# HaSai666/rec_pangu

Hardware: AMD Instinct MI355X
Metric: samples/sec DeepFM Criteo-shape bsz=65536/GPU (train step: fwd+bwd+dense Adam+zero_grad) (higher is better)
Workload: dtype f32

## Files before the change

### include/rec_pangu_hip.h

```cpp
#ifndef REC_PANGU_HIP_H
#define REC_PANGU_HIP_H

#include <stddef.h>
#include <stdint.h>

#ifdef __cplusplus
extern "C" {
#endif

#define RP_OK 0
#define RP_ERR_ARG (-1)
#define RP_ERR_LAUNCH (-2)
#define RP_ERR_UNSUPPORTED (-3)

#define RP_MAX_FIELDS 64

#define RP_ACT_NONE 0
#define RP_ACT_RELU 1
#define RP_ACT_MASK 2
#define RP_ACT_TANH 3
#define RP_ACT_SIGMOID 4
#define RP_ACT_LEAKY 5

#define RP_MATMUL_FP32 0
#define RP_MATMUL_BF16 1
#define RP_MATMUL_AUTO 2
#define RP_MATMUL_BF16X3 3
#define RP_MATMUL_BF16X6 6
int rp_set_matmul_precision(int mode);
int rp_get_matmul_precision(void);

typedef void *rp_stream_t;

#define RP_ABI_VERSION 108
int rp_version(void);
const char *rp_last_error(void);
uint64_t rp_launch_count(void);

int rp_embed_gather_fwd(const float *arena, const int64_t *row_base, const int64_t *row_count,
                        const int64_t *const *idx_ptrs, int F, const float *const *dense_ptrs, int ND,
                        int64_t B, int D, float *x, int64_t ldx, float *fm_out, float *sum_out,
                        int32_t *keys_out, int32_t *err_flag, rp_stream_t stream);

int rp_embed_gather_linear_fits(int D, int ND, int hidden, int64_t ldx, int64_t ldw);
int rp_embed_gather_linear_fwd(const float *arena, const int64_t *row_base, const int64_t *row_count,
                               const int64_t *const *idx_ptrs, int F, const float *const *dense_ptrs, int ND, int64_t B,
                               int D, float *x, int64_t ldx, const float *W, int64_t ldw, const float *bias, float *h1,
                               float *fm_out, float *sum_out, int32_t *keys_out, int32_t *err_flag, float *xd, rp_stream_t stream);
int rp_embed_gather_linear_fwd_bf16(const void *arena_bf16, const int64_t *row_base, const int64_t *row_count,
                                    const int64_t *const *idx_ptrs, int F, const float *const *dense_ptrs, int ND, int64_t B,
                                    int D, const float *W, int64_t ldw, const float *bias, float *h1, float *fm_out,
                                    void *x_bf16, int64_t ldx, float *sum_out, int32_t *keys_out, int32_t *err_flag,
                                    float *xd, rp_stream_t stream);

int rp_sort_workspace_bytes(int64_t n, size_t *bytes);
int rp_sort_pairs_i32(void *workspace, size_t workspace_bytes, const int32_t *keys_in, int32_t *keys_out,
                      int32_t *pos_out, int64_t n, int end_bit, rp_stream_t stream);
int rp_sort_pairs_fields_workspace_bytes(int64_t B, int F, size_t *bytes);
int rp_sort_pairs_fields_i32(void *workspace, size_t workspace_bytes, const int32_t *keys_in, int32_t *keys_out,
                             int32_t *pos_out, int64_t B, int F, const int64_t *field_base, const int64_t *field_rows,
                             rp_stream_t stream);
int rp_embed_grad_reduce_workspace_bytes(int64_t n, int D, size_t *bytes);
int rp_embed_grad_reduce(const int32_t *sorted_keys, const int32_t *sorted_pos, int64_t n, int64_t B, int D,
                         const float *dx, int64_t ldx, const float *gfm, const float *sum_in,
                         const float *arena, float *grad_arena, int accumulate, void *workspace,
                         size_t workspace_bytes, rp_stream_t stream);
int rp_embed_grad_gemm_fits(int D, int hidden, int64_t lddh, int64_t ldwt);
int rp_embed_grad_gemm(const int32_t *sorted_keys, const int32_t *sorted_pos, int64_t n, int64_t B, int D, const float *dh,
                       int64_t lddh, const float *wt, int64_t ldwt, const float *dx, int64_t ldx, const float *gfm,
                       const float *sum_in, const float *arena, float *grad_arena, int accumulate, uint64_t skip_fields,
                       void *workspace, size_t workspace_bytes, rp_stream_t stream);
int rp_embed_grad_tiny_workspace_bytes(int64_t B, size_t *bytes);
int rp_embed_grad_tiny(const int32_t *keys, int64_t B, const int32_t *tiny_field, const int64_t *tiny_base,
                       const int32_t *tiny_rows, int n_tiny, const float *dh, int64_t lddh, const float *wt, int64_t ldwt,
                       const float *gfm, const float *sum_in, const float *arena, float *grad_arena, int accumulate,
                       float *dw, int64_t lddw, void *workspace, size_t workspace_bytes, rp_stream_t stream);
int rp_embed_grad_seg_fits(int D, int hidden, int64_t lddh);
int rp_embed_grad_seg_workspace_bytes(int64_t n, int64_t B, int D, size_t *bytes);
int rp_embed_grad_seg(const int32_t *sorted_keys, const int32_t *sorted_pos, int64_t n, int64_t B, int D, const float *dh,
                      int64_t lddh, const float *w, int64_t ldw, const float *gfm, const float *sum_in, const float *arena,
                      float *grad_arena, int accumulate, uint64_t skip_fields, const int64_t *field_rows, float *dw,
                      int64_t lddw, void *workspace, size_t workspace_bytes, rp_stream_t stream);
int rp_embed_grad_ss_workspace_bytes(int64_t n, int64_t B, int D, uint64_t skip_fields, size_t *bytes);
int rp_embed_grad_ss_mark_sizes(int64_t B, int n_kept, size_t *n_rows, size_t *n_offs);
int rp_embed_grad_ss_mark(const int32_t *sorted_keys, int64_t n, int64_t B, uint64_t skip_fields, int32_t *ustart, int32_t *ukey,
                          int32_t *offs, rp_stream_t stream);
int rp_embed_grad_ss(const int32_t *sorted_keys, const int32_t *sorted_pos, int64_t n, int64_t B, int D, const float *dh,
                     int64_t lddh, const float *w, int64_t ldw, const float *gfm, const float *sum_in, const float *arena,
                     float *grad_arena, int accumulate, uint64_t skip_fields, const int64_t *field_rows, float *dw,
                     int64_t lddw, const int32_t *ustart, const int32_t *ukey, const int32_t *offs, int phases,
                     void *workspace, size_t workspace_bytes, rp_stream_t stream);
int rp_embed_grad_smp_fits(int D, int hidden, int64_t lddh);
int rp_embed_grad_smp_workspace_bytes(int64_t B, int n_fields, size_t *bytes);
int rp_embed_grad_smp_mark_scratch(int64_t B, int n_fields, size_t *n_int32);
int rp_embed_grad_smp_mark(const int32_t *sorted_keys, const int32_t *sorted_pos, int64_t n, int64_t B,
                           const int32_t *fields, int n_fields, int32_t *dupq, int32_t *dupkeys, int32_t *scratch,
                           rp_stream_t stream);
int rp_embed_grad_smp(const int32_t *keys, const int32_t *dupq, const int32_t *dupkeys, int64_t B, int F,
                      const int32_t *fields, const int64_t *field_base, const int64_t *field_rows, int n_fields,
                      const float *dh, int64_t lddh, const float *w, int64_t ldw,
                      const float *gfm, const float *sum_in, const float *arena, float *grad_arena, int accumulate,
                      float *dw, int64_t lddw, int phases, void *workspace, size_t workspace_bytes, rp_stream_t stream);
int rp_embed_grad_reduce_rows(const int32_t *keys, const float *rows, int64_t n, int D, float *grad_arena, int accumulate,
                              void *workspace, size_t workspace_bytes, rp_stream_t stream);
int rp_zero_rows(const int32_t *keys, int64_t n, int D, float *grad_arena, rp_stream_t stream);
int rp_fill_words(void *dst, int64_t n_words, uint32_t value, rp_stream_t stream);

int rp_linear_fwd(const float *a, int64_t lda, const float *w, int64_t ldw, const float *bias, float *out,
                  int64_t ldo, int64_t M, int N, int K, int act, const float *aux, int64_t ldaux,
                  rp_stream_t stream);
int rp_linear_wgrad_workspace_bytes(int64_t M, int N, int K, size_t *bytes);
int rp_linear_wgrad(const float *dy, int64_t lddy, const float *x, int64_t ldx, float *dw, int64_t lddw,
                    float *db, int64_t M, int N, int K, int accumulate, void *workspace,
                    size_t workspace_bytes, rp_stream_t stream);
int rp_linear_wgrad_xbf16(const float *dy, int64_t lddy, const void *x_bf16, int64_t ldx, float *dw, int64_t lddw,
                          float *db, int64_t M, int N, int K, int accumulate, void *workspace, size_t workspace_bytes,
                          rp_stream_t stream);
int rp_transpose(const float *in, int64_t ldin, float *out, int64_t ldout, int R, int C, int C_out, rp_stream_t stream);
int rp_transpose_copy(const float *in, int64_t ldin, float *out, int64_t ldout, int R, int C, int C_out, float *copy,
                      int64_t ldcopy, rp_stream_t stream);
int rp_copy_rows(const float *in, int64_t ldin, float *out, int64_t ldout, int R, int C, rp_stream_t stream);
int rp_add_rows(const float *in, int64_t ldin, float *out, int64_t ldout, int R, int C, rp_stream_t stream);
int64_t rp_pieces_ld(int K, int np);
int rp_pieces_pack(const float *in, int64_t ld, int64_t M, int K, int np, void *out, int64_t ldo, rp_stream_t stream);
int rp_linear_fwd_pieces(const void *a, int64_t lda, const void *w, int64_t ldw, const float *bias, float *out,
                         int64_t ldo, int64_t M, int N, int K, int np, int act, const float *aux, int64_t ldaux,
                         rp_stream_t stream);
int rp_relu_bwd(const float *dy, int64_t lddy, const float *act_out, int64_t ldact, float *out, int64_t ldo,
                int64_t M, int N, rp_stream_t stream);
int rp_act_fwd(const float *x, int64_t ldx, float *y, int64_t ldy, int64_t M, int N, int act, rp_stream_t stream);
int rp_act_bwd(const float *dy, int64_t lddy, const float *act_out, int64_t ldact, float *out, int64_t ldo, int64_t M,
               int N, int act, rp_stream_t stream);

int rp_crossnet_fwd(const float *x0, int64_t ldx, int d, int L, const float *W, const float *Bv, const float *wfc,
                    const float *bfc, float *xout, int64_t ldo, float *logit, float *s_out, int64_t B,
                    rp_stream_t stream);

int rp_cin_layer_fwd(const float *x0, int64_t ld0, const float *xp, int64_t ldp, const float *W, const float *bias,
                     float *out, float *pooled, int64_t ldpool, int H, int M, int O, int D, int64_t B,
                     rp_stream_t stream);
int rp_cin_layer_bwd_x(const float *x0, int64_t ld0, const float *xp, int64_t ldp, const float *W, const float *g_out,
                       const float *g_pool, int64_t ldgp, float *dx0, int64_t lddx0, int add_dx0, float *dxp,
                       int64_t lddxp, int H, int M, int O, int D, int64_t B, rp_stream_t stream);
int rp_cin_layer_bwd_w_workspace_bytes(int64_t B, int H, int M, int O, size_t *bytes);
int rp_cin_layer_bwd_w(const float *x0, int64_t ld0, const float *xp, int64_t ldp, const float *g_out,
                       const float *g_pool, int64_t ldgp, float *dW, float *dbias, int H, int M, int O, int D,
                       int64_t B, void *workspace, size_t workspace_bytes, rp_stream_t stream);

int rp_field_attention_fits(int T, int Din, int H, int a, int has_res);
int rp_field_attention_fwd(const float *x, int64_t ldx, const float *W, int T, int Din, int H, int a, int has_res,
                           float scale, float *out, int64_t B, rp_stream_t stream);
int rp_field_attention_bwd_workspace_bytes(int64_t B, int T, int Din, int H, int a, int has_res, size_t *bytes);
int rp_field_attention_bwd(const float *x, int64_t ldx, const float *W, int T, int Din, int H, int a, int has_res,
                           float scale, const float *gout, float *dx, int64_t lddx, float *dW, int64_t B,
                           void *workspace, size_t workspace_bytes, rp_stream_t stream);

int rp_mmoe_combine_fwd(const float *z, int64_t ldz, int K, int E, int T, float *out, float *gate, int64_t B,
                        rp_stream_t stream);
int rp_mmoe_combine_bwd(const float *z, int64_t ldz, int K, int E, int T, const float *gate, const float *dout,
                        float *dz, int64_t lddz, int64_t B, rp_stream_t stream);

int rp_crossnet_bwd_rows(const float *x0, int64_t ldx, int d, int L, const float *W, const float *wfc,
                         const float *s_in, const float *g_x, int64_t ldg, const float *g_logit, float *dx0,
                         int64_t lddx, float *V, int64_t B, rp_stream_t stream);
int rp_crossnet_param_grads(const float *P, int64_t ldp, const float *cs, const float *W, const float *Bv, const float *wfc,
                            const float *colg, int L, int d, float *dW, float *dB, float *dwfc, rp_stream_t stream);

int rp_cin_bs_fits(int H, int M, int D);
int rp_accumulate(float *dst, const float *src, int64_t n, rp_stream_t stream);
int rp_cin_bs_fwd(const float *x0, int64_t ld0, const float *xp, int64_t ldp, const void *wp, const float *bias, int H,
                  int M, int O, int D, float *out, float *pooled, int64_t B, rp_stream_t stream);
int rp_cin_bs_bwd_x(const float *xk, int64_t ldk, const void *wp, const float *gout, const float *gpool, int R, int Cn,
                    int O, int D, float *dx, int64_t lddx, int64_t B, rp_stream_t stream);
int rp_cin_bs_bwd_w_workspace_bytes(int64_t B, int O, size_t *bytes);
int rp_cin_bs_bwd_w(const float *x0, int64_t ld0, const float *xp, int64_t ldp, const float *gout, const float *gpool,
                    int H, int M, int O, int D, float *dW, float *db, int64_t B, void *workspace, size_t workspace_bytes,
                    rp_stream_t stream);
int rp_cin_pair_fits(int H, int O, int D);
int rp_cin_pair_fwd(const float *x0, int64_t ld0, const void *wsp, const float *bias, int H, int O, int D, float *out,
                    float *pooled, int64_t B, rp_stream_t stream);
int rp_cin_pair_bwd_x(const float *x0, int64_t ld0, const void *wst, const float *gout, const float *gpool,
                      const int32_t *lstart, const int32_t *lent, int H, int O, int D, float *dx, int64_t lddx, int64_t B,
                      int accumulate, rp_stream_t stream);
int rp_cin_pair_bwd_w_workspace_bytes(int64_t B, int H, int O, size_t *bytes);
int rp_cin_pair_bwd_w(const float *x0, int64_t ld0, const float *gout, const float *gpool, int H, int O, int D, float *dW,
                      float *db, int64_t B, void *workspace, size_t workspace_bytes, rp_stream_t stream);

int rp_cin_last_fits(int H, int M, int D);
int rp_cin_last_fwd(const float *x0, int64_t ld0, const float *xp, int64_t ldp, const float *vt, int H, int M, int D,
                    float *pooled, int64_t B, rp_stream_t stream);
int rp_cin_last_bwd_x(const float *x0, int64_t ld0, const float *xp, int64_t ldp, const float *vt, const float *g, int H,
                      int M, int D, float *dx0, int64_t ldd0, float *dxp, int64_t lddp, int64_t B, rp_stream_t stream);
int rp_cin_last_bwd_v_workspace_bytes(int64_t B, int H, int M, size_t *bytes);
int rp_cin_last_bwd_v(const float *x0, int64_t ld0, const float *xp, int64_t ldp, const float *g, int H, int M, int D,
                      float *dV, int64_t B, void *workspace, size_t workspace_bytes, rp_stream_t stream);
int rp_cin_pair_pieces(const float *W, int O, int H, void *wsp, void *wst, rp_stream_t stream);
int rp_cin_head_params_fwd(const float *WL, const float *bL, const float *c, int O, int H, int M, float *vt, float *vb,
                           rp_stream_t stream);
int rp_cin_head_params_bwd(const float *WL, const float *bL, const float *c, const float *dV, const float *sg, float Dscale,
                           int O, int H, int M, float *dWL, float *dbL, float *dc, rp_stream_t stream);
int rp_add_scalars(float *out, int64_t n, const float *a, float scale, const float *b0, rp_stream_t stream);
int rp_sum_all(const float *x, int64_t n, float *out, rp_stream_t stream);

// ... 336 lines not shown
```

### rec_pangu_amd/csrc/common.h

```cpp
#pragma once
#include <hip/hip_runtime.h>
#include <stdint.h>
#include <stddef.h>
#include "../../include/rec_pangu_hip.h"

#include <string.h>
#include <tuple>
#include <utility>

int rp_fail(int code, const char *fmt, ...);
void rp_count_launch();

#define RP_MAX_KERNARG 4096
bool rp_plan_recording();
void rp_plan_record(const void *func, dim3 grid, dim3 block, unsigned shmem, hipStream_t stream, const char *blob,
                    size_t blob_bytes, const size_t *offsets, int nargs);

template <typename T>
static inline size_t rp_pack_arg(char *buf, size_t &off, const T &v) {
    off = (off + alignof(T) - 1) & ~(size_t)(alignof(T) - 1);
    const size_t at = off;
    memcpy(buf + at, &v, sizeof(T));
    off += sizeof(T);
    return at;
}

template <size_t I, typename K, typename Tup>
static inline K rp_arg_or_zero(Tup &t) {
    if constexpr (I < std::tuple_size<Tup>::value) return static_cast<K>(std::get<I>(t));
    else return K{};
}

template <typename... KArgs, typename Tup, size_t... I>
static inline void rp_launch_packed(void (*kernel)(KArgs...), dim3 grid, dim3 block, unsigned shmem, hipStream_t stream,
                                    Tup &args, std::index_sequence<I...>) {
    constexpr int N = (int)sizeof...(KArgs);
    static_assert((sizeof(KArgs) + ... + 0) + 16 * sizeof...(KArgs) <= RP_MAX_KERNARG, "kernel arguments exceed the packing buffer");
    alignas(16) char buf[RP_MAX_KERNARG];
    size_t off = 0;
    size_t offs[N ? N : 1] = {rp_pack_arg<KArgs>(buf, off, rp_arg_or_zero<I, KArgs>(args))...};
    void *ptrs[N ? N : 1];
    for (int i = 0; i < N; ++i) ptrs[i] = buf + offs[i];
    if (rp_plan_recording()) rp_plan_record(reinterpret_cast<const void *>(kernel), grid, block, shmem, stream, buf, off, offs, N);
    (void)hipLaunchKernel(reinterpret_cast<const void *>(kernel), grid, block, ptrs, shmem, stream);
}

template <typename... KArgs, typename... Args>
static inline void rp_launch(void (*kernel)(KArgs...), dim3 grid, dim3 block, unsigned shmem, hipStream_t stream,
                             Args &&...args) {
    static_assert(sizeof...(Args) <= sizeof...(KArgs), "kernel launch: too many arguments");
    auto tup = std::forward_as_tuple(std::forward<Args>(args)...);
    rp_launch_packed(kernel, grid, block, shmem, stream, tup, std::make_index_sequence<sizeof...(KArgs)>());
}

#undef hipLaunchKernelGGL
#define hipLaunchKernelGGL(kernel, grid, block, shmem, stream, ...) rp_launch(kernel, grid, block, shmem, stream, __VA_ARGS__)

#define RP_REQUIRE(cond, ...)                                  \
    do {                                                       \
        if (!(cond)) return rp_fail(RP_ERR_ARG, __VA_ARGS__);  \
    } while (0)

#define RP_LAUNCH_CHECK(name)                                                        \
    do {                                                                             \
        hipError_t e__ = hipGetLastError();                                          \
        if (e__ != hipSuccess)                                                       \
            return rp_fail(RP_ERR_LAUNCH, "%s: %s", name, hipGetErrorString(e__));   \
        rp_count_launch();                                                           \
    } while (0)

static inline bool rp_aligned16(const void *p) { return (reinterpret_cast<uintptr_t>(p) & 15u) == 0; }
static inline int64_t rp_cdiv(int64_t a, int64_t b) { return (a + b - 1) / b; }

typedef float f32x4 __attribute__((ext_vector_type(4)));
typedef float f32x16 __attribute__((ext_vector_type(16)));

__device__ __forceinline__ float rp_act_apply(int act, float v) {
    switch (act) {
        case RP_ACT_RELU: return v > 0.f ? v : 0.f;
        case RP_ACT_TANH: return tanhf(v);
        case RP_ACT_SIGMOID: return 1.f / (1.f + expf(-v));
        case RP_ACT_LEAKY: return v > 0.f ? v : 0.01f * v;
        default: return v;
    }
}
__device__ __forceinline__ float rp_act_grad(int act, float dy, float y) {
    switch (act) {
        case RP_ACT_RELU: return y > 0.f ? dy : 0.f;
        case RP_ACT_TANH: return dy * (1.f - y * y);
        case RP_ACT_SIGMOID: return dy * (y * (1.f - y));
        case RP_ACT_LEAKY: return y > 0.f ? dy : 0.01f * dy;
        default: return dy;
    }
}

#define RP_WAVE 64

int rp_matmul_products(double flops, double bytes);

int rp_int_grad_reduce_finish(int64_t n, int D, int64_t nb0, char *wbase, float *piece0, int32_t *key0, float *grad_arena,
                              int accumulate, hipStream_t s);
```

### rec_pangu_amd/csrc/embed.hip

```cpp
#include "common.h"
#include <cstdlib>
#include "bfsplit.h"

struct IdxPtrs {
    const int64_t *p[RP_MAX_FIELDS];
};
struct DensePtrs {
    const float *p[RP_MAX_FIELDS];
};

template <int VEC>
struct Vec;
template <>
struct Vec<4> {
    typedef f32x4 T;
    static __device__ __forceinline__ T load(const float *p) { return *reinterpret_cast<const f32x4 *>(p); }
    static __device__ __forceinline__ void store(float *p, T v) { *reinterpret_cast<f32x4 *>(p) = v; }
    static __device__ __forceinline__ T zero() { return f32x4{0.f, 0.f, 0.f, 0.f}; }
    static __device__ __forceinline__ float hsum(T v) { return (v.x + v.y) + (v.z + v.w); }
};
template <>
struct Vec<1> {
    typedef float T;
    static __device__ __forceinline__ T load(const float *p) { return *p; }
// ... 150 lines not shown
                    gs = 0.f;
                    run_head = true;
                }
            }
        }
        __syncthreads();
        if (grp == 0) {
            const bool head_open = pkey[0][0] >= 0;
            int last_g = -1;
            for (int g2 = GPB - 1; g2 >= 0; --g2)
                if (pkey[g2][0] >= 0 || pkey[g2][1] >= 0) {
                    last_g = g2;
                    break;
                }
            const int64_t wg_end = ((int64_t)blockIdx.x + 1) * GPB * RP_SEG;
            const int last_active = (int)(((n < wg_end ? n : wg_end) - (int64_t)blockIdx.x * GPB * RP_SEG + RP_SEG - 1) / RP_SEG) - 1;
            const bool tail_open = last_g >= 0 && last_g == last_active && pcont[last_g] != 0;
            int32_t cur = -1;
            bool cur_is_head = false;
            typename V::T cacc = V::zero();
            int32_t headkey = -1, tailkey = -1;
            typename V::T headv = V::zero(), tailv = V::zero();
            for (int g2 = 0; g2 < GPB; ++g2) {
#pragma unroll
                for (int slot = 0; slot < 2; ++slot) {
                    const int32_t key = pkey[g2][slot];
                    if (key < 0) continue;
                    const typename V::T pv = V::load(&piece[g2][slot][t * VEC]);
                    if (key == cur) {
                        cacc += pv;
                    } else {
                        if (cur >= 0) {
                            if (cur_is_head) {
                                headkey = cur;
                                headv = cacc;
                            } else if (col_ok) {
                                float *dst = G + (int64_t)cur * D + c;
                                V::store(dst, accumulate ? V::load(dst) + cacc : cacc);
                            }
                        }
                        cur = key;
                        cacc = pv;
                        cur_is_head = head_open && g2 == 0 && slot == 0;
                    }
                }
            }
            if (cur >= 0) {
                if (tail_open) {
                    if (cur_is_head) {
                        headkey = cur;
                        headv = cacc;
                        tailkey = cur;
                    } else {
                        tailkey = cur;
                        tailv = cacc;
                    }
                } else if (cur_is_head) {
                    headkey = cur;
                    headv = cacc;
                } else if (col_ok) {
                    float *dst = G + (int64_t)cur * D + c;
                    V::store(dst, accumulate ? V::load(dst) + cacc : cacc);
                }
            }
            if (col_ok) {
                V::store(hp + c, headv);
                V::store(tp + c, tailv);
            }
            if (t == 0 && c0 == 0) {
                gkey[2 * (int64_t)blockIdx.x] = headkey;
                gkey[2 * (int64_t)blockIdx.x + 1] = tailkey;
            }
        }
        __syncthreads();
    }
}

#define EG_LD 72
#define EG_CT 68
#define EGL_MAXF 32

#define EGL_XLD 68
#define EGL_KLD 33
template <bool FULL, bool STORE_X = true, bool BF16_ROWS = false>
__global__ __launch_bounds__(256, 2) void embed_gather_linear_kernel(
    const float *__restrict__ arena, const int64_t *__restrict__ row_base, const int64_t *__restrict__ row_count,
    IdxPtrs idx, int F, DensePtrs dense, int ND, int64_t B, int64_t blk0, float *__restrict__ x, int64_t ldx,
    const float *__restrict__ W, int64_t ldw, const float *__restrict__ bias, float *__restrict__ h1,
    float *__restrict__ fm_out, float *__restrict__ sum_out, int32_t *__restrict__ keys_out, int32_t *__restrict__ err_flag,
    float *__restrict__ xd) {
    constexpr int D = 64;
    __shared__ __attribute__((aligned(16))) __bf16 Wt[3][64][EG_LD];
    __shared__ __attribute__((aligned(16))) float Xs[128][EGL_XLD];
    __shared__ int32_t Ks[128][EGL_KLD];
    const int t = threadIdx.x;
    const int wv = t >> 6, l = t & 63, i = l & 31, h = l >> 5;
    const int64_t blk = blk0 + blockIdx.x;
    const int64_t b = blk * 128 + 32 * wv + i;
    const bool bok = FULL || b < B;
    const int64_t bc = bok ? b : B - 1;
    const int g = t >> 4, sub = t & 15;
    const int wd = t >> 2, wc = (t & 3) * 16;

    for (int f = h; f < F; f += 2) {
        int64_t id = idx.p[f][bc];
        if (id < 0 || id >= row_count[f]) {
            if (bok) *err_flag = 1;
            id = 0;
        }
        const int64_t key = row_base[f] + id;
        Ks[32 * wv + i][f] = (int32_t)key;
        if (keys_out != nullptr && bok) keys_out[(int64_t)f * B + b] = (int32_t)key;
    }
    __syncthreads();
    const int g8 = t >> 3, s8 = t & 7;
    auto row_of = [&](int u) { return BF16_ROWS ? g8 + 32 * (u >> 1) : g + 16 * u; };
    auto col_of = [&](int u) { return BF16_ROWS ? 8 * s8 + 4 * (u & 1) : 4 * sub; };
    auto load_rows = [&](int f, f32x4 (&v)[8]) {
        if (BF16_ROWS) {
#pragma unroll
            for (int u = 0; u < 4; ++u) {
                const uint4 w4 = *reinterpret_cast<const uint4 *>(reinterpret_cast<const uint16_t *>(arena) +
                                                                  (int64_t)Ks[g8 + 32 * u][f] * D + 8 * s8);
                v[2 * u] = f32x4{__uint_as_float(w4.x << 16), __uint_as_float(w4.x & 0xffff0000u),
                                 __uint_as_float(w4.y << 16), __uint_as_float(w4.y & 0xffff0000u)};
                v[2 * u + 1] = f32x4{__uint_as_float(w4.z << 16), __uint_as_float(w4.z & 0xffff0000u),
                                     __uint_as_float(w4.w << 16), __uint_as_float(w4.w & 0xffff0000u)};
            }
        } else {
#pragma unroll
            for (int u = 0; u < 8; ++u) v[u] = *reinterpret_cast<const f32x4 *>(arena + (int64_t)Ks[g + 16 * u][f] * D + 4 * sub);
        }
    };
    auto load_w = [&](int col0, f32x4 (&v)[4]) {
        const float *src = W + (int64_t)wd * ldw + col0 + wc;
#pragma unroll
        for (int u = 0; u < 4; ++u) v[u] = *reinterpret_cast<const f32x4 *>(src + 4 * u);
    };
    f32x16 acc[2];
#pragma unroll
    for (int nt = 0; nt < 2; ++nt)
#pragma unroll
        for (int r = 0; r < 16; ++r) acc[nt][r] = 0.f;
    f32x4 S[8];
    float q[8];
#pragma unroll
    for (int u = 0; u < 8; ++u) {
        S[u] = f32x4{0.f, 0.f, 0.f, 0.f};
        q[u] = 0.f;
    }
    f32x4 cur[8], nxt[8], wq[4], wqn[4];
    load_rows(0, cur);
    load_w(0, wq);
    for (int f = 0; f < F; ++f) {
        const int fn = f + 1 < F ? f + 1 : f;
        load_rows(fn, nxt);
        load_w(fn * D, wqn);
        __syncthreads();
#pragma unroll
        for (int u = 0; u < 8; ++u) {
            const int r = row_of(u);
            *reinterpret_cast<f32x4 *>(&Xs[r][col_of(u)]) = cur[u];
            const int64_t br = blk * 128 + r;
            if (STORE_X && (FULL || (x != nullptr && br < B))) {
                if (BF16_ROWS) {
                    uint2 w2;
                    w2.x = (__float_as_uint(cur[u][0]) >> 16) | (__float_as_uint(cur[u][1]) & 0xFFFF0000u);
                    w2.y = (__float_as_uint(cur[u][2]) >> 16) | (__float_as_uint(cur[u][3]) & 0xFFFF0000u);
                    *reinterpret_cast<uint2 *>(reinterpret_cast<uint16_t *>(x) + br * ldx + (int64_t)f * D + col_of(u)) = w2;
                } else {
                    *reinterpret_cast<f32x4 *>(x + br * ldx + (int64_t)f * D + col_of(u)) = cur[u];
                }
            }
            S[u] += cur[u];
#pragma unroll
            for (int e = 0; e < 4; ++e) q[u] = __builtin_fmaf(cur[u][e], cur[u][e], q[u]);
        }
#pragma unroll
        for (int u = 0; u < 2; ++u) {
            f32x8 v;
#pragma unroll
            for (int e = 0; e < 4; ++e) {
                v[e] = wq[2 * u][e];
                v[4 + e] = wq[2 * u + 1][e];
            }
            bf16x8 pc[3];
            bf_split8<3>(v, pc);
#pragma unroll
            for (int qq = 0; qq < 3; ++qq) *reinterpret_cast<bf16x8 *>(&Wt[qq][wd][wc + 8 * u]) = pc[qq];
        }
        __syncthreads();
#pragma unroll
        for (int ks = 0; ks < 4; ++ks) {
            const f32x4 v0 = *reinterpret_cast<const f32x4 *>(&Xs[32 * wv + i][ks * 16 + 8 * h]);
            const f32x4 v1 = *reinterpret_cast<const f32x4 *>(&Xs[32 * wv + i][ks * 16 + 8 * h + 4]);
            f32x8 av;
#pragma unroll
            for (int e = 0; e < 4; ++e) {
                av[e] = v0[e];
                av[4 + e] = v1[e];
            }
            bf16x8 a[3];
            bf_split8<3>(av, a);
#pragma unroll
            for (int nt = 0; nt < 2; ++nt) {
                bf16x8 bq[3];
#pragma unroll
                for (int qq = 0; qq < 3; ++qq) bq[qq] = *reinterpret_cast<const bf16x8 *>(&Wt[qq][nt * 32 + i][ks * 16 + 8 * h]);
#pragma unroll
                for (int pr = 0; pr < 6; ++pr) {
                    if (BF16_ROWS && BfProd<6>::pa(pr) != 0) continue;
                    acc[nt] = __builtin_amdgcn_mfma_f32_32x32x16_bf16(a[BfProd<6>::pa(pr)], bq[BfProd<6>::pb(pr)], acc[nt], 0, 0, 0);
                }
            }
        }
#pragma unroll
        for (int u = 0; u < 8; ++u) cur[u] = nxt[u];
#pragma unroll
        for (int u = 0; u < 4; ++u) wq[u] = wqn[u];
    }
    if (ND > 0) {
        __syncthreads();
        {
#pragma unroll
            for (int u = 0; u < 4; ++u) {
                const int e = (t & 3) * 4 + u;
                const float v = e < ND ? W[(int64_t)wd * ldw + (int64_t)F * D + e] : 0.f;
                const __bf16 hi = (__bf16)v;
                const float r1 = v - (float)hi;
                const __bf16 mid = (__bf16)r1;
                Wt[0][wd][e] = hi;
                Wt[1][wd][e] = mid;
                Wt[2][wd][e] = (__bf16)(r1 - (float)mid);
            }
        }
        f32x8 dv;
#pragma unroll
        for (int e = 0; e < 8; ++e) {
            const int k = 8 * h + e;
            dv[e] = k < ND ? dense.p[k][bc] : 0.f;
        }
        __syncthreads();
        if (x != nullptr && bok && BF16_ROWS) {
            uint16_t *xt = reinterpret_cast<uint16_t *>(x) + b * ldx + (int64_t)F * D;
#pragma unroll
            for (int e = 0; e < 8; ++e)
                if (8 * h + e < ND) {
                    uint32_t ub = __float_as_uint(dv[e]);
                    ub += 0x7FFFu + ((ub >> 16) & 1u);
                    xt[8 * h + e] = (uint16_t)(ub >> 16);
                }
            for (int64_t j = (int64_t)F * D + ND + h; j < ldx; j += 2) reinterpret_cast<uint16_t *>(x)[b * ldx + j] = 0;
        } else if (x != nullptr && bok) {
            float *xt = x + b * ldx + (int64_t)F * D;
#pragma unroll
            for (int e = 0; e < 8; ++e)
                if (8 * h + e < ND) xt[8 * h + e] = dv[e];
            for (int64_t j = (int64_t)F * D + ND + h; j < ldx; j += 2) x[b * ldx + j] = 0.f;
        }
        if (xd != nullptr && bok) {
            float *xt = xd + b * 64;
#pragma unroll
            for (int e = 0; e < 8; ++e) xt[8 * h + e] = (8 * h + e < ND) ? dv[e] : 0.f;
            for (int j = 16 + h; j < 64; j += 2) xt[j] = 0.f;
        }
        bf16x8 a[3];
        bf_split8<3>(dv, a);
#pragma unroll
        for (int nt = 0; nt < 2; ++nt) {
            bf16x8 bq[3];
#pragma unroll
            for (int qq = 0; qq < 3; ++qq) bq[qq] = *reinterpret_cast<const bf16x8 *>(&Wt[qq][nt * 32 + i][8 * h]);
#pragma unroll
            for (int pr = 0; pr < 6; ++pr)
                acc[nt] = __builtin_amdgcn_mfma_f32_32x32x16_bf16(a[BfProd<6>::pa(pr)], bq[BfProd<6>::pb(pr)], acc[nt], 0, 0, 0);
        }
    } else {
        if (x != nullptr && bok && BF16_ROWS)
            for (int64_t j = (int64_t)F * D + h; j < ldx; j += 2) reinterpret_cast<uint16_t *>(x)[b * ldx + j] = 0;
        else if (x != nullptr && bok)
            for (int64_t j = (int64_t)F * D + h; j < ldx; j += 2) x[b * ldx + j] = 0.f;
        if (xd != nullptr && bok)
            for (int j = h; j < 64; j += 2) xd[b * 64 + j] = 0.f;
    }
#pragma unroll
    for (int nt = 0; nt < 2; ++nt) {
        const int n = nt * 32 + i;
        const float bv = bias != nullptr ? bias[n] : 0.f;
#pragma unroll
        for (int r = 0; r < 16; ++r) {
            const int64_t m = blk * 128 + 32 * wv + (r & 3) + 8 * (r >> 2) + 4 * h;
            if (FULL || m < B) h1[m * 64 + n] = fmaxf(acc[nt][r] + bv, 0.f);
        }
    }
    if (BF16_ROWS) {
#pragma unroll
        for (int u = 0; u < 4; ++u) {
            const int64_t br = blk * 128 + g8 + 32 * u;
            float fmv = -(q[2 * u] + q[2 * u + 1]);
#pragma unroll
            for (int e = 0; e < 4; ++e) {
                fmv = __builtin_fmaf(S[2 * u][e], S[2 * u][e], fmv);
                fmv = __builtin_fmaf(S[2 * u + 1][e], S[2 * u + 1][e], fmv);
            }
            fmv += __shfl_xor(fmv, 1, 64);
            fmv += __shfl_xor(fmv, 2, 64);
            fmv += __shfl_xor(fmv, 4, 64);
            if ((FULL || br < B) && fm_out != nullptr && s8 == 0) fm_out[br] = 0.5f * fmv;
            if ((FULL || br < B) && sum_out != nullptr) {
                *reinterpret_cast<f32x4 *>(sum_out + br * D + 8 * s8) = S[2 * u];
                *reinterpret_cast<f32x4 *>(sum_out + br * D + 8 * s8 + 4) = S[2 * u + 1];
            }
        }
        return;
    }
#pragma unroll
    for (int u = 0; u < 8; ++u) {
        const int64_t br = blk * 128 + g + 16 * u;
        float fmv = -q[u];
#pragma unroll
        for (int e = 0; e < 4; ++e) fmv = __builtin_fmaf(S[u][e], S[u][e], fmv);
        fmv += __shfl_xor(fmv, 1, 64);
        fmv += __shfl_xor(fmv, 2, 64);
        fmv += __shfl_xor(fmv, 4, 64);
        fmv += __shfl_xor(fmv, 8, 64);
        if (FULL || br < B) {
            if (fm_out != nullptr && sub == 0) fm_out[br] = 0.5f * fmv;
            if (sum_out != nullptr) *reinterpret_cast<f32x4 *>(sum_out + br * D + 4 * sub) = S[u];
        }
    }
}

static int embed_gather_linear_launch(const float *arena, bool bf16_rows, const int64_t *row_base, const int64_t *row_count,
                                      const int64_t *const *idx_ptrs, int F, const float *const *dense_ptrs, int ND,
                                      int64_t B, int D, float *x, int64_t ldx, const float *W, int64_t ldw,
                                      const float *bias, float *h1, float *fm_out, float *sum_out, int32_t *keys_out,
                                      int32_t *err_flag, float *xd, rp_stream_t stream);

extern "C" int rp_embed_gather_linear_fits(int D, int ND, int hidden, int64_t ldx, int64_t ldw) {
    return (D == 64 && hidden == 64 && ND >= 0 && ND <= 16 && ldx % 4 == 0 && ldw % 4 == 0) ? 1 : 0;
}

extern "C" int rp_embed_gather_linear_fwd(const float *arena, const int64_t *row_base, const int64_t *row_count,
                                          const int64_t *const *idx_ptrs, int F, const float *const *dense_ptrs, int ND,
                                          int64_t B, int D, float *x, int64_t ldx, const float *W, int64_t ldw,
                                          const float *bias, float *h1, float *fm_out, float *sum_out, int32_t *keys_out,
                                          int32_t *err_flag, float *xd, rp_stream_t stream) {
    return embed_gather_linear_launch(arena, false, row_base, row_count, idx_ptrs, F, dense_ptrs, ND, B, D, x, ldx, W, ldw, bias,
                                      h1, fm_out, sum_out, keys_out, err_flag, xd, stream);
}

extern "C" int rp_embed_gather_linear_fwd_bf16(const void *arena_bf16, const int64_t *row_base, const int64_t *row_count,
                                               const int64_t *const *idx_ptrs, int F, const float *const *dense_ptrs, int ND,
                                               int64_t B, int D, const float *W, int64_t ldw, const float *bias, float *h1,
                                               float *fm_out, void *x_bf16, int64_t ldx, float *sum_out, int32_t *keys_out,
                                               int32_t *err_flag, float *xd, rp_stream_t stream) {
    RP_REQUIRE(x_bf16 == nullptr || (ldx % 4 == 0 && (reinterpret_cast<uintptr_t>(x_bf16) & 7u) == 0),
               "embed_gather_linear_fwd_bf16: the bf16 activation needs ldx %% 4 == 0 and 8-byte alignment");
    return embed_gather_linear_launch(reinterpret_cast<const float *>(arena_bf16), true, row_base, row_count, idx_ptrs, F,
                                      dense_ptrs, ND, B, D, reinterpret_cast<float *>(x_bf16), ldx, W, ldw, bias, h1, fm_out,
                                      sum_out, keys_out, err_flag, xd, stream);
}

static int embed_gather_linear_launch(const float *arena, bool bf16_rows, const int64_t *row_base, const int64_t *row_count,
                                      const int64_t *const *idx_ptrs, int F, const float *const *dense_ptrs, int ND,
                                      int64_t B, int D, float *x, int64_t ldx, const float *W, int64_t ldw,
                                      const float *bias, float *h1, float *fm_out, float *sum_out, int32_t *keys_out,
                                      int32_t *err_flag, float *xd, rp_stream_t stream) {
    RP_REQUIRE(arena && row_base && row_count && idx_ptrs && W && h1 && err_flag, "embed_gather_linear_fwd: null pointer");
    RP_REQUIRE(!(x && xd), "embed_gather_linear_fwd: give x (full activation) or xd (dense columns only), not both");
    RP_REQUIRE(F >= 1 && F <= RP_MAX_FIELDS && B >= 0, "embed_gather_linear_fwd: bad F/B");
    RP_REQUIRE(ND == 0 || dense_ptrs, "embed_gather_linear_fwd: dense_ptrs is null with ND=%d", ND);
    RP_REQUIRE((int64_t)F * B < (int64_t)INT32_MAX, "embed_gather_linear_fwd: F*B overflows int32 positions");
    if (F > EGL_MAXF || !rp_embed_gather_linear_fits(D, ND, 64, x ? ldx : 4, ldw) || !rp_aligned16(arena) || !rp_aligned16(W) ||
        (x && (!rp_aligned16(x) || ldx < (int64_t)F * D + ND)) || ldw < (int64_t)F * D + ND ||
        (sum_out && !rp_aligned16(sum_out)))
        return rp_fail(RP_ERR_UNSUPPORTED, "embed_gather_linear_fwd: needs D = 64, a 64-wide layer, ND <= 16, aligned operands");
    if (B == 0) return RP_OK;
    IdxPtrs ip;
    DensePtrs dp;
    for (int f = 0; f < F; ++f) {
        RP_REQUIRE(idx_ptrs[f], "embed_gather_linear_fwd: idx_ptrs[%d] is null", f);
        ip.p[f] = idx_ptrs[f];
    }
    for (int j = 0; j < ND; ++j) {
        RP_REQUIRE(dense_ptrs[j], "embed_gather_linear_fwd: dense_ptrs[%d] is null", j);
        dp.p[j] = dense_ptrs[j];
    }
    const int64_t nfull = B / 128;
    const int64_t nblk = rp_cdiv(B, 128);
    hipStream_t s = (hipStream_t)stream;
    if (bf16_rows) {
        if (nfull > 0 && x != nullptr)
            hipLaunchKernelGGL((embed_gather_linear_kernel<true, true, true>), dim3((unsigned)nfull), dim3(256), 0, s, arena,
                               row_base, row_count, ip, F, dp, ND, B, (int64_t)0, x, ldx, W, ldw, bias, h1, fm_out, sum_out,
                               keys_out, err_flag, xd);
        else if (nfull > 0)
            hipLaunchKernelGGL((embed_gather_linear_kernel<true, false, true>), dim3((unsigned)nfull), dim3(256), 0, s, arena,
                               row_base, row_count, ip, F, dp, ND, B, (int64_t)0, x, ldx, W, ldw, bias, h1, fm_out, sum_out,
                               keys_out, err_flag, xd);
        if (nblk > nfull)
            hipLaunchKernelGGL((embed_gather_linear_kernel<false, true, true>), dim3((unsigned)(nblk - nfull)), dim3(256), 0, s,
                               arena, row_base, row_count, ip, F, dp, ND, B, nfull, x, ldx, W, ldw, bias, h1, fm_out, sum_out,
                               keys_out, err_flag, xd);
        RP_LAUNCH_CHECK("embed_gather_linear_fwd (bf16 rows)");
        return RP_OK;
    }
    if (nfull > 0 && x != nullptr)
        hipLaunchKernelGGL((embed_gather_linear_kernel<true, true>), dim3((unsigned)nfull), dim3(256), 0, s, arena, row_base,
                           row_count, ip, F, dp, ND, B, (int64_t)0, x, ldx, W, ldw, bias, h1, fm_out, sum_out, keys_out, err_flag,
                           xd);
    else if (nfull > 0)
        hipLaunchKernelGGL((embed_gather_linear_kernel<true, false>), dim3((unsigned)nfull), dim3(256), 0, s, arena, row_base,
                           row_count, ip, F, dp, ND, B, (int64_t)0, x, ldx, W, ldw, bias, h1, fm_out, sum_out, keys_out, err_flag,
                           xd);
    if (nblk > nfull)
        hipLaunchKernelGGL((embed_gather_linear_kernel<false, true>), dim3((unsigned)(nblk - nfull)), dim3(256), 0, s, arena,
                           row_base, row_count, ip, F, dp, ND, B, nfull, x, ldx, W, ldw, bias, h1, fm_out, sum_out, keys_out,
                           err_flag, xd);
    RP_LAUNCH_CHECK("embed_gather_linear_fwd");
    return RP_OK;
}

#define EG_MAXG 34
struct GradRanges {
    int n;
    int64_t start[EG_MAXG], end[EG_MAXG];
    int tile0[EG_MAXG];
};

template <bool FM_U>
__global__ __launch_bounds__(256, 3) void embed_grad_gemm_kernel(
    const int32_t *__restrict__ sk, const int32_t *__restrict__ sp, int64_t n, int Bi, const float *__restrict__ dh,
    int64_t lddh, const float *__restrict__ wt, int64_t ldwt, const float *__restrict__ dx, int64_t ldx,
    const float *__restrict__ gfm, const float *__restrict__ sum_in, const float *__restrict__ arena,
    float *__restrict__ G, int accumulate, float *__restrict__ gpiece, int32_t *__restrict__ gkey, GradRanges rg) {
    typedef Vec<4> V;
    constexpr int D = 64, TPR = 16, VEC = 4, GPB = 16, W = 64;
    constexpr int SM_B = 3 * 64 * EG_LD * 2, SM_C = 128 * EG_CT * 4;
    __shared__ __attribute__((aligned(16))) char smem[SM_B > SM_C ? SM_B : SM_C];
    __shared__ __attribute__((aligned(16))) float piece[GPB][2][W];
    __shared__ int32_t pkey[GPB][2];
    __shared__ int32_t pcont[GPB];
    __shared__ int32_t tkey[130];
    __shared__ int32_t tsmp[128];
    __shared__ int32_t tfld[128];
    __shared__ float tgf[128];
    typedef __bf16(*BTile)[64][EG_LD];
    BTile Bt = reinterpret_cast<BTile>(smem);
    float(*Ct)[EG_CT] = reinterpret_cast<float(*)[EG_CT]>(smem);
    const int t = threadIdx.x % TPR, grp = threadIdx.x / TPR;
    int gi = 0;
    for (int g2 = 1; g2 < rg.n; ++g2)
        if ((int)blockIdx.x >= rg.tile0[g2]) gi = g2;
    const int64_t wg0 = rg.start[gi] + (int64_t)((int)blockIdx.x - rg.tile0[gi]) * GPB * RP_SEG;
    const int64_t gend = rg.end[gi];
    {
        const int wv = threadIdx.x >> 6, l = threadIdx.x & 63, i = l & 31, h = l >> 5;
        const int64_t prow = wg0 + 32 * wv + i;
        const bool rok = prow < gend;
        const int32_t pp = rok ? sp[prow] : 0;
        const int32_t kk = rok ? sk[prow] : -1;
        if (threadIdx.x == 0) tkey[0] = wg0 > 0 ? sk[wg0 - 1] : -1;
        if (threadIdx.x == 64) tkey[129] = wg0 + 128 < n ? sk[wg0 + 128] : -1;
        const int fr = pp / Bi, br = pp - fr * Bi;
        const int64_t plast = (wg0 + 127 < gend ? wg0 + 127 : gend - 1);
        const int f_lo = __builtin_amdgcn_readfirstlane(sp[wg0] / Bi), f_hi = __builtin_amdgcn_readfirstlane(sp[plast] / Bi);
        if (h == 0) {
            tkey[1 + 32 * wv + i] = kk;
            tsmp[32 * wv + i] = br;
            tfld[32 * wv + i] = fr;
        }
        const bool wrap = __syncthreads_or(rok && (fr < f_lo || fr > f_hi)) != 0;
        const float gme = (gfm != nullptr && rok) ? gfm[br] : 0.f;
        f32x4 araw[4][2];
        const float *asrc = dh + (int64_t)br * lddh + 8 * h;
#pragma unroll
        for (int ks = 0; ks < 4; ++ks) {
            araw[ks][0] = *reinterpret_cast<const f32x4 *>(asrc + ks * 16);
            araw[ks][1] = *reinterpret_cast<const f32x4 *>(asrc + ks * 16 + 4);
        }
        float uraw[2][16];
        if (FM_U) {
#pragma unroll
            for (int r = 0; r < 16; ++r) {
                const float *src = sum_in + (int64_t)tsmp[32 * wv + (r & 3) + 8 * (r >> 2) + 4 * h] * D + i;
                uraw[0][r] = src[0];
                uraw[1][r] = src[32];
            }
        }
        if (h == 0) tgf[32 * wv + i] = gme;
        f32x16 acc[2];
#pragma unroll
        for (int nt = 0; nt < 2; ++nt)
#pragma unroll
            for (int r = 0; r < 16; ++r) acc[nt][r] = 0.f;
        const int wd = threadIdx.x >> 2, wc = (threadIdx.x & 3) * 16;
        const int f_from = wrap ? 0 : f_lo, f_to = wrap ? (int)((n - 1) / Bi) : f_hi;
        bool first_pass = true, need_init = FM_U;
        for (int f = f_from; f <= f_to; ++f) {
            if (wrap && !__syncthreads_or(rok && fr == f)) continue;
// ... 1003 lines not shown
```

### rec_pangu_amd/csrc/gemm.hip

```cpp
#include "common.h"
#include <cstdlib>

#define BM 128
#define BN 64
#define BK 32
#define LDS_LD 36

__device__ __forceinline__ f32x4 load4_guard(const float *p, int valid, bool vec) {
    if (vec && valid >= 4) return *reinterpret_cast<const f32x4 *>(p);
    f32x4 v = {0.f, 0.f, 0.f, 0.f};
    if (valid > 0) v.x = p[0];
    if (valid > 1) v.y = p[1];
    if (valid > 2) v.z = p[2];
    if (valid > 3) v.w = p[3];
    return v;
}

template <bool VEC_A, bool VEC_W>
__global__ __launch_bounds__(256) void linear_fwd_kernel(const float *__restrict__ A, int64_t lda,
                                                         const float *__restrict__ W, int64_t ldw,
                                                         const float *__restrict__ bias, float *__restrict__ C,
                                                         int64_t ldc, int64_t M, int N, int K, int act,
                                                         const float *__restrict__ aux, int64_t ldaux) {
    __shared__ __attribute__((aligned(16))) float smem[(BM + BN) * LDS_LD];
// ... 826 lines not shown
#pragma unroll
        for (int p = 0; p < PF; ++p) load_tile_full((int64_t)p * TN_BM, ry[p], rx[p]);
        const int64_t nloop = (nstf - PF) / PF;
        for (int64_t it = 0; it < nloop; ++it) {
#pragma unroll
            for (int p = 0; p < PF; ++p) {
                stage(ry[p], rx[p]);
                load_tile_full((it * PF + p + PF) * TN_BM, ry[p], rx[p]);
                compute();
            }
        }
        sbeg = nloop * PF;
    } else {
#pragma unroll
        for (int p = 0; p < PF; ++p)
            if (p < nst) load_tile(mbeg + (int64_t)p * TN_BM, ry[p], rx[p]);
    }
    for (int64_t s0 = sbeg; s0 < nst; s0 += PF) {
#pragma unroll
        for (int p = 0; p < PF; ++p) {
            const int64_t st = s0 + p;
            if (st >= nst) break;
            stage(ry[p], rx[p]);
            if (st + PF < nst) load_tile(mbeg + (st + PF) * TN_BM, ry[p], rx[p]);
            compute();
        }
    }
    float *Pz = P + (int64_t)bz * N * K;
#pragma unroll
    for (int u = 0; u < NA; ++u)
#pragma unroll
        for (int kk = 0; kk < 2; ++kk) {
            const int k = k0 + kt + kk * 32 + i;
            if (k >= K) continue;
#pragma unroll
            for (int r = 0; r < 16; ++r) {
                const int n = n0 + nt + 32 * u + (r & 3) + 8 * (r >> 2) + 4 * h;
                if (n < N) Pz[(int64_t)n * K + k] = acc[u][kk][r];
            }
        }
    if (do_bias) {
#pragma unroll
        for (int u = 0; u < NA; ++u) bred[o][c + 64 * u] = bsum[u];
        __syncthreads();
        for (int e = t; e < BNT; e += 256)
            if (n0 + e < N) Pb[(int64_t)bz * N + n0 + e] = (bred[0][e] + bred[1][e]) + (bred[2][e] + bred[3][e]);
    }
}

__global__ __launch_bounds__(256) void wgrad_reduce_kernel(const float *__restrict__ P, const float *__restrict__ Pb,
                                                           int S, int N, int K, float *__restrict__ dw,
                                                           int64_t lddw, float *__restrict__ db, int accumulate) {
    __shared__ float red[16][17];
    const int c = threadIdx.x & 15, q = threadIdx.x >> 4;
    const int64_t e = (int64_t)blockIdx.x * 16 + c;
    const int64_t nk = (int64_t)N * K;
    const bool is_w = e < nk, is_b = !is_w && e < nk + N && db != nullptr;
    float s = 0.f;
    if (is_w) {
#pragma unroll 4
        for (int z = q; z < S; z += 16) s += P[(int64_t)z * nk + e];
    } else if (is_b) {
        const int n = (int)(e - nk);
#pragma unroll 4
        for (int z = q; z < S; z += 16) s += Pb[(int64_t)z * N + n];
    }
    red[q][c] = s;
    __syncthreads();
    if (q != 0) return;
#pragma unroll
    for (int j = 1; j < 16; ++j) s += red[j][c];
    if (is_w) {
        const int n = (int)(e / K), k = (int)(e - (int64_t)n * K);
        float *d = dw + (int64_t)n * lddw + k;
        *d = accumulate ? (*d + s) : s;
    } else if (is_b) {
        const int n = (int)(e - nk);
        db[n] = accumulate ? (db[n] + s) : s;
    }
}

__global__ __launch_bounds__(256) void transpose_kernel(const float *__restrict__ in, int64_t ldin,
                                                        float *__restrict__ out, int64_t ldout, int R, int C, int C_out,
                                                        float *__restrict__ copy = nullptr, int64_t ldcopy = 0) {
    __shared__ float tile[32][33];
    const int tx = threadIdx.x & 31, ty = threadIdx.x >> 5;
    const int c0 = blockIdx.x * 32, r0 = blockIdx.y * 32;
#pragma unroll
    for (int j = 0; j < 32; j += 8) {
        const int r = r0 + ty + j, c = c0 + tx;
        const bool ok = r < R && c < C;
        const float v = ok ? in[(int64_t)r * ldin + c] : 0.f;
        tile[ty + j][tx] = v;
        if (copy != nullptr && ok) copy[(int64_t)r * ldcopy + c] = v;
    }
    __syncthreads();
#pragma unroll
    for (int j = 0; j < 32; j += 8) {
        const int c = c0 + ty + j, r = r0 + tx;
        if (r < R && c < C_out) out[(int64_t)c * ldout + r] = tile[tx][ty + j];
    }
}

__global__ __launch_bounds__(256) void relu_bwd_kernel(const float *__restrict__ dy, int64_t lddy,
                                                       const float *__restrict__ y, int64_t ldy,
                                                       float *__restrict__ out, int64_t ldo, int64_t M, int N) {
    const int64_t total = M * N;
    for (int64_t e = (int64_t)blockIdx.x * blockDim.x + threadIdx.x; e < total; e += (int64_t)gridDim.x * blockDim.x) {
        const int64_t m = e / N;
        const int n = (int)(e - m * N);
        out[m * ldo + n] = (y[m * ldy + n] > 0.f) ? dy[m * lddy + n] : 0.f;
    }
}

template <int NPROD>
static void launch_smallk_rowadd(const float *a, int64_t lda, const float *w, int64_t ldw, float *out, int64_t ldo,
                                 int64_t M, int N, int K, const float *rs, const float *radd, int64_t ldadd, int nadd,
                                 hipStream_t s) {
    const int64_t mb = M / 128;
    const int tiles = N / BN;
    int64_t ysplit = rp_cdiv(768, mb);
    if (ysplit > tiles) ysplit = tiles;
    if (ysplit < 1) ysplit = 1;
    const int per = (int)rp_cdiv(tiles, ysplit);
    dim3 grid((unsigned)mb, (unsigned)rp_cdiv(tiles, per));
    hipLaunchKernelGGL((linear_fwd_bf16_smallk_kernel<NPROD, RP_ACT_NONE, true, true>), grid, dim3(256), 0, s, a, lda, w, ldw,
                       nullptr, out, ldo, M, N, K, nullptr, 0, per, rs, radd, ldadd, nadd);
}

static int g_matmul_precision = RP_MATMUL_AUTO;

extern "C" int rp_set_matmul_precision(int mode) {
    RP_REQUIRE(mode == RP_MATMUL_FP32 || mode == RP_MATMUL_BF16 || mode == RP_MATMUL_BF16X3 || mode == RP_MATMUL_BF16X6 ||
                   mode == RP_MATMUL_AUTO, "set_matmul_precision: unknown mode %d", mode);
    g_matmul_precision = mode;
    return RP_OK;
}

int rp_matmul_products(double flops, double bytes) {
    switch (g_matmul_precision) {
        case RP_MATMUL_FP32: return 0;
        case RP_MATMUL_BF16: return 1;
        case RP_MATMUL_BF16X3: return 3;
        case RP_MATMUL_BF16X6: return 6;
        default: break;
    }
    return (bytes > 0 && flops * 3.0 / bytes > 312.0) ? 3 : 6;
}

static int linear_mode(int64_t M, int N, int K) {
    if (g_matmul_precision != RP_MATMUL_AUTO) return g_matmul_precision;
    return rp_matmul_products(2.0 * M * N * K, 4.0 * ((double)M * K + (double)N * K + (double)M * N)) == 3
               ? RP_MATMUL_BF16X3 : RP_MATMUL_BF16X6;
}

extern "C" int rp_get_matmul_precision(void) { return g_matmul_precision; }

extern "C" int rp_linear_fwd_rowadd(const float *a, int64_t lda, const float *w, int64_t ldw, float *out, int64_t ldo,
                                    int64_t M, int N, int K, const float *row_scale, const float *row_add,
                                    int64_t ld_add, int add_cols, rp_stream_t stream) {
    RP_REQUIRE(a && w && out && row_scale && row_add, "linear_fwd_rowadd: null pointer");
    RP_REQUIRE(lda >= K && ldw >= K && ldo >= N && ld_add >= 64, "linear_fwd_rowadd: leading dimension too small");
    const int mode = linear_mode(M, N, K);
    const bool ok = mode != RP_MATMUL_FP32 && K >= 4 && K <= 64 && K % 4 == 0 && M >= 128 && M % 128 == 0 && N >= 64 &&
                    N % 64 == 0 && add_cols >= 0 && add_cols % 64 == 0 && add_cols <= N && lda % 4 == 0 && ldw % 4 == 0 &&
                    rp_aligned16(a) && rp_aligned16(w);
    if (!ok) return rp_fail(RP_ERR_UNSUPPORTED, "linear_fwd_rowadd: shape/alignment/mode outside the fused kernel");
    hipStream_t s = (hipStream_t)stream;
// ... 175 lines not shown
        RP_LAUNCH_CHECK("linear_wgrad partial (bf16 split)");
    } else {
#define CALL(VY, VX)                                                                                                \
    hipLaunchKernelGGL((linear_wgrad_partial_kernel<VY, VX>), grid, dim3(256), 0, s, dy, lddy, x, ldx, P, Pb, M, N, K, \
                       rows)
    if (vy && vx) CALL(true, true);
    else if (vy) CALL(true, false);
    else if (vx) CALL(false, true);
    else CALL(false, false);
#undef CALL
    RP_LAUNCH_CHECK("linear_wgrad partial");
    }
    const int64_t total = (int64_t)N * K + N;
    hipLaunchKernelGGL(wgrad_reduce_kernel, dim3((unsigned)rp_cdiv(total, 16)), dim3(256), 0, s, P, Pb, S, N, K, dw,
                       lddw, db, accumulate);
    RP_LAUNCH_CHECK("linear_wgrad reduce");
    return RP_OK;
}

extern "C" int rp_linear_wgrad_xbf16(const float *dy, int64_t lddy, const void *x_bf16, int64_t ldx, float *dw, int64_t lddw,
                                     float *db, int64_t M, int N, int K, int accumulate, void *workspace,
                                     size_t workspace_bytes, rp_stream_t stream) {
    RP_REQUIRE(dy && x_bf16 && dw && workspace, "linear_wgrad_xbf16: null pointer");
    RP_REQUIRE(M >= 1 && N >= 1 && K >= 1, "linear_wgrad_xbf16: bad M/N/K");
    RP_REQUIRE(lddy >= N && ldx >= K && lddw >= K, "linear_wgrad_xbf16: leading dimension too small");
    const int mode = linear_mode(M, N, K);
    if (mode == RP_MATMUL_FP32 || wgrad_wide(N) || ldx % 2 != 0 || (reinterpret_cast<uintptr_t>(x_bf16) & 3u) != 0)
        return rp_fail(RP_ERR_UNSUPPORTED, "linear_wgrad_xbf16: bf16 matrix-core modes, N <= 128, ldx even, 4-byte aligned x only");
    size_t need = 0;
    rp_linear_wgrad_workspace_bytes(M, N, K, &need);
    RP_REQUIRE(workspace_bytes >= need, "linear_wgrad_xbf16: workspace %zu < %zu bytes", workspace_bytes, need);
    int S;
    int64_t rows;
    wgrad_plan(M, N, K, &S, &rows);
    float *P = reinterpret_cast<float *>((reinterpret_cast<uintptr_t>(workspace) + 255) & ~(uintptr_t)255);
    float *Pb = P + (size_t)S * N * K;
    dim3 gridb((unsigned)rp_cdiv(K, TN_BK), (unsigned)rp_cdiv(N, TN_BN), (unsigned)S);
    hipStream_t s = (hipStream_t)stream;
    const float *xf = reinterpret_cast<const float *>(x_bf16);
#define CALLX(NPROD)                                                                                                       \
    hipLaunchKernelGGL((linear_wgrad_bf16_kernel<NPROD, 1, 1, true, true>), gridb, dim3(256), 0, s, dy, lddy, xf, ldx, P, Pb, M, \
                       N, K, rows, 0, 0, S)
    if (mode == RP_MATMUL_BF16X6) CALLX(6);
    else if (mode == RP_MATMUL_BF16X3) CALLX(3);
    else CALLX(1);
#undef CALLX
    RP_LAUNCH_CHECK("linear_wgrad_xbf16 partial");
    const int64_t total = (int64_t)N * K + N;
    hipLaunchKernelGGL(wgrad_reduce_kernel, dim3((unsigned)rp_cdiv(total, 16)), dim3(256), 0, s, P, Pb, S, N, K, dw, lddw, db,
                       accumulate);
    RP_LAUNCH_CHECK("linear_wgrad_xbf16 reduce");
    return RP_OK;
}

extern "C" int rp_transpose(const float *in, int64_t ldin, float *out, int64_t ldout, int R, int C, int C_out,
                            rp_stream_t stream) {
    RP_REQUIRE(in && out && R >= 1 && C >= 1 && C_out >= C && ldin >= C && ldout >= R, "transpose: bad argument");
    dim3 grid((unsigned)rp_cdiv(C_out, 32), (unsigned)rp_cdiv(R, 32));
    hipLaunchKernelGGL(transpose_kernel, grid, dim3(256), 0, (hipStream_t)stream, in, ldin, out, ldout, R, C, C_out);
    RP_LAUNCH_CHECK("transpose");
    return RP_OK;
}

__global__ __launch_bounds__(256) void copy_rows_kernel(const float *__restrict__ in, int64_t ldin, float *__restrict__ out,
                                                        int64_t ldout, int R, int C) {
    const int64_t total = (int64_t)R * C;
    for (int64_t e = (int64_t)blockIdx.x * 256 + threadIdx.x; e < total; e += (int64_t)gridDim.x * 256) {
        const int64_t r = e / C;
        const int c = (int)(e - r * C);
        out[r * ldout + c] = in[r * ldin + c];
    }
}

extern "C" int rp_transpose_copy(const float *in, int64_t ldin, float *out, int64_t ldout, int R, int C, int C_out,
                                 float *copy, int64_t ldcopy, rp_stream_t stream) {
    RP_REQUIRE(in && out && copy && R >= 1 && C >= 1 && C_out >= C && ldin >= C && ldout >= R && ldcopy >= C,
               "transpose_copy: bad argument");
    const dim3 grid((unsigned)rp_cdiv(C_out, 32), (unsigned)rp_cdiv(R, 32));
    hipLaunchKernelGGL(transpose_kernel, grid, dim3(256), 0, (hipStream_t)stream, in, ldin, out, ldout, R, C, C_out, copy, ldcopy);
    RP_LAUNCH_CHECK("transpose_copy");
    return RP_OK;
}

extern "C" int rp_copy_rows(const float *in, int64_t ldin, float *out, int64_t ldout, int R, int C, rp_stream_t stream) {
    RP_REQUIRE(in && out && R >= 1 && C >= 1 && ldin >= C && ldout >= C, "copy_rows: bad argument");
    int64_t blocks = rp_cdiv((int64_t)R * C, 256);
    if (blocks > 2048) blocks = 2048;
    hipLaunchKernelGGL(copy_rows_kernel, dim3((unsigned)blocks), dim3(256), 0, (hipStream_t)stream, in, ldin, out, ldout, R, C);
    RP_LAUNCH_CHECK("copy_rows");
    return RP_OK;
}

__global__ __launch_bounds__(256) void add_rows_kernel(const float *__restrict__ in, int64_t ldin, float *__restrict__ out,
                                                       int64_t ldout, int R, int C) {
    const int64_t total = (int64_t)R * C;
    for (int64_t e = (int64_t)blockIdx.x * 256 + threadIdx.x; e < total; e += (int64_t)gridDim.x * 256) {
        const int64_t r = e / C;
        const int c = (int)(e - r * C);
        out[r * ldout + c] += in[r * ldin + c];
    }
}

extern "C" int rp_add_rows(const float *in, int64_t ldin, float *out, int64_t ldout, int R, int C, rp_stream_t stream) {
    RP_REQUIRE(in && out && R >= 1 && C >= 1 && ldin >= C && ldout >= C, "add_rows: bad argument");
    int64_t blocks = rp_cdiv((int64_t)R * C, 256);
    if (blocks > 4096) blocks = 4096;
    hipLaunchKernelGGL(add_rows_kernel, dim3((unsigned)blocks), dim3(256), 0, (hipStream_t)stream, in, ldin, out, ldout, R, C);
    RP_LAUNCH_CHECK("add_rows");
    return RP_OK;
}

__global__ __launch_bounds__(256) void act_fwd_kernel(const float *__restrict__ x, int64_t ldx, float *__restrict__ y,
                                                      int64_t ldy, int64_t M, int N, int act) {
    const int64_t total = M * N;
    for (int64_t e = (int64_t)blockIdx.x * 256 + threadIdx.x; e < total; e += (int64_t)gridDim.x * 256) {
        const int64_t r = e / N;
        const int c = (int)(e - r * N);
        y[r * ldy + c] = rp_act_apply(act, x[r * ldx + c]);
    }
}

__global__ __launch_bounds__(256) void act_bwd_kernel(const float *__restrict__ dy, int64_t lddy, const float *__restrict__ ya,
                                                      int64_t ldact, float *__restrict__ out, int64_t ldo, int64_t M, int N,
                                                      int act) {
    const int64_t total = M * N;
    for (int64_t e = (int64_t)blockIdx.x * 256 + threadIdx.x; e < total; e += (int64_t)gridDim.x * 256) {
        const int64_t r = e / N;
        const int c = (int)(e - r * N);
        out[r * ldo + c] = rp_act_grad(act, dy[r * lddy + c], ya[r * ldact + c]);
    }
}

static bool act_kind_ok(int act) { return act == RP_ACT_RELU || act == RP_ACT_TANH || act == RP_ACT_SIGMOID || act == RP_ACT_LEAKY; }

extern "C" int rp_act_fwd(const float *x, int64_t ldx, float *y, int64_t ldy, int64_t M, int N, int act, rp_stream_t stream) {
    RP_REQUIRE(x && y && M >= 0 && N >= 1 && ldx >= N && ldy >= N && act_kind_ok(act), "act_fwd: bad argument");
    if (M == 0) return RP_OK;
    int64_t blocks = rp_cdiv(M * N, 256);
    if (blocks > 4096) blocks = 4096;
    hipLaunchKernelGGL(act_fwd_kernel, dim3((unsigned)blocks), dim3(256), 0, (hipStream_t)stream, x, ldx, y, ldy, M, N, act);
    RP_LAUNCH_CHECK("act_fwd");
    return RP_OK;
}

extern "C" int rp_act_bwd(const float *dy, int64_t lddy, const float *act_out, int64_t ldact, float *out, int64_t ldo,
                          int64_t M, int N, int act, rp_stream_t stream) {
    RP_REQUIRE(dy && act_out && out && M >= 0 && N >= 1 && act_kind_ok(act), "act_bwd: bad argument");
    if (M == 0) return RP_OK;
    int64_t blocks = rp_cdiv(M * N, 256);
    if (blocks > 4096) blocks = 4096;
    hipLaunchKernelGGL(act_bwd_kernel, dim3((unsigned)blocks), dim3(256), 0, (hipStream_t)stream, dy, lddy, act_out, ldact, out, ldo,
                       M, N, act);
    RP_LAUNCH_CHECK("act_bwd");
    return RP_OK;
}

extern "C" int rp_relu_bwd(const float *dy, int64_t lddy, const float *act_out, int64_t ldact, float *out,
                           int64_t ldo, int64_t M, int N, rp_stream_t stream) {
    RP_REQUIRE(dy && act_out && out && M >= 0 && N >= 1, "relu_bwd: bad argument");
    if (M == 0) return RP_OK;
    int64_t blocks = rp_cdiv(M * N, 256);
    if (blocks > 4096) blocks = 4096;
    hipLaunchKernelGGL(relu_bwd_kernel, dim3((unsigned)blocks), dim3(256), 0, (hipStream_t)stream, dy, lddy, act_out,
                       ldact, out, ldo, M, N);
    RP_LAUNCH_CHECK("relu_bwd");
    return RP_OK;
// ... 2 lines not shown
```

### rec_pangu_amd/functional.py

```python
import contextlib
import os
from typing import List, NamedTuple, Optional, Sequence, Tuple

import torch

from . import hip

ACT_NONE, ACT_RELU, ACT_MASK = hip.ACT_NONE, hip.ACT_RELU, hip.ACT_MASK
ACT_TANH, ACT_SIGMOID, ACT_LEAKY = hip.ACT_TANH, hip.ACT_SIGMOID, hip.ACT_LEAKY


def act_code(module):
    import torch.nn as nn
    if isinstance(module, nn.ReLU):
        return ACT_RELU
    if isinstance(module, nn.Tanh):
        return ACT_TANH
    if isinstance(module, nn.Sigmoid):
        return ACT_SIGMOID
    if isinstance(module, nn.LeakyReLU) and abs(module.negative_slope - 0.01) < 1e-12:
        return ACT_LEAKY
    return None


def _unit_inner(t: torch.Tensor) -> torch.Tensor:
    if t.dim() == 2 and (t.shape[1] <= 1 or t.stride(1) == 1) and (t.shape[0] <= 1 or t.stride(0) >= t.shape[1]):
        return t
    return t.contiguous()


def padded(width: int, pad_to: int) -> int:
    return width if pad_to <= 1 else (width + pad_to - 1) // pad_to * pad_to


def _wide_rows_grad(rows: torch.Tensor, used: int) -> Optional[torch.Tensor]:
    return hip.zeros(tuple(rows.shape), torch.float32, rows.device) if rows.shape[1] > used else None


def _rows16(w: torch.Tensor) -> torch.Tensor:
    K = w.shape[1]
    if K % 4 == 0 or K <= 64 or not w.is_cuda:
        return w
    key = (w.data_ptr(), w._version, hip.weight_epoch(), torch.cuda.is_current_stream_capturing())
    hit = getattr(w, "_rp_rows16", None)
    if hit is not None and hit[0] == key:
        return hit[1]
    with torch.no_grad():
        if w.dtype is torch.float32:
            out = hip.copy_rows(w.detach(), (K + 3) // 4 * 4)
        else:
            buf = torch.empty((w.shape[0], (K + 3) // 4 * 4), dtype=w.dtype, device=w.device)
            buf[:, :K].copy_(w)
            out = buf[:, :K]
    if not key[3]:
        try:
            w._rp_rows16 = (key, out)
        except AttributeError:
            pass
    return out


class FMFold:
    __slots__ = ("ssum", "ncols", "dfm", "folded", "dgrad", "D", "fused", "extra")

    def __init__(self, ssum, ncols, D=0):
        self.ssum, self.ncols, self.dfm, self.folded = ssum, ncols, None, False
        self.extra = None
        self.dgrad, self.D, self.fused = None, D, False


class _TokenView(torch.autograd.Function):

    @staticmethod
    def forward(ctx, x, F: int, D: int, link):
        x = _unit_inner(x)
        out = torch.empty((x.shape[0], F * D), dtype=torch.float32, device=x.device)
        hip.copy_rows_to(x[:, :F * D], out)
        ctx.link = link
        return out.view(x.shape[0], F, D)

    @staticmethod
    def backward(ctx, dtok):
        ctx.link.extra = dtok.reshape(dtok.shape[0], -1).contiguous()
        return None, None, None, None


def token_view(x, F: int, D: int, link):
    return _TokenView.apply(x, F, D, link)


class _StackRows(torch.autograd.Function):

    @staticmethod
    def forward(ctx, *ws):
        rows = [w.shape[0] for w in ws]
        out = torch.empty((sum(rows), ws[0].shape[1]), dtype=torch.float32, device=ws[0].device)
        dst, r0 = [], 0
        for r in rows:
            dst.append(out[r0:r0 + r])
            r0 += r
        src = [w.detach().contiguous() for w in ws]
        if not hip.multi_copy(dst, src):
            torch._foreach_copy_(dst, src)
        ctx.rows = rows
        return out

    @staticmethod
    def backward(ctx, g):
        g = g.contiguous()
        outs, r0 = [], 0
        for r in ctx.rows:
            outs.append(g[r0:r0 + r])
            r0 += r
        return tuple(outs)


def stack_rows(ws):
    return _StackRows.apply(*ws)


class _GradTap(torch.autograd.Function):

    @staticmethod
    def forward(ctx, t, link):
        ctx.link = link
        return t.view_as(t)

    @staticmethod
    def backward(ctx, g):
        ctx.link.dfm = g
        return g, None


def tap_fm_grad(fm, link):
    return _GradTap.apply(fm, link)


class ReluLink:
    __slots__ = ("dx",)
# ... 1245 lines not shown
        store._presorted = None
        row_base, row_count = meta if meta is not None else (store.row_base, store.row_count)
        x, fm, ssum, keys = hip.embed_gather_fwd(store.arena, row_base, row_count, idx, dense, ldx,
                                                 want_fm, want_fm and need_grad, need_grad and pre is None,
                                                 store.err_flag)
        ctx.store, ctx.want_fm, ctx.B = store, want_fm, idx[0].shape[0]
        ctx.link = store._fm_link = FMFold(ssum, len(idx) * store.embedding_dim, store.embedding_dim) \
            if (need_grad and meta is None) else None
        ctx.presorted = pre if need_grad else None
        if pre is not None:
            keys = pre.keys if need_grad else None
        ctx.save_for_backward(keys, ssum)
        if want_fm:
            return x, fm
        return x

    @staticmethod
    def backward(ctx, dx, dfm=None):
        keys, ssum = ctx.saved_tensors
        store = ctx.store
        fused = None
        if ctx.link is not None and ctx.link.dgrad is not None:
            fused, ctx.link.dgrad = ctx.link.dgrad, None
            ctx.link.fused = True
            if dx is not None and dx.dim() == 2 and dx.stride(0) == 0 and dx.stride(1) == 0:
                dx = None
        if dx is not None:
            dx = _unit_inner(dx)
        if ctx.link is not None and ctx.link.extra is not None:
            extra, ctx.link.extra = ctx.link.extra, None
            if fused is not None and dx is None and extra.shape[1] == len(store.emb_feature) * store.embedding_dim:
                dx = extra
            elif dx is None or fused is not None:
                raise RuntimeError("token_view: the gathered activation needs a consumer that materialises its gradient")
            else:
                hip.add_rows_to(extra, dx[:, :extra.shape[1]])
        gfm = dfm.contiguous() if (ctx.want_fm and dfm is not None) else None
        if ctx.link is not None and ctx.link.folded:
            ssum = None
        if fused is None:
            store.accumulate_grad(keys, ctx.B, dx, gfm, ssum, presorted=ctx.presorted)
        else:
            g = store.first_layer_grad(keys, ctx.B, *fused, gfm, ssum, presorted=ctx.presorted, dx=dx)
            if g.forms.tiny:
                g.tiny()
            g.gemm()
            g.done()
        return (None,) * (6 + len(store.emb_feature))


_WGRAD_STREAMS: dict = {}


def _side2_stream(device):
    st = _WGRAD_STREAMS.get(device)
    if st is None:
        st = _WGRAD_STREAMS[device] = hip.make_side_stream(device)
    return st


def _masked_by_consumer(lk, dy) -> bool:
    masked = lk is not None and lk.dx is not None and lk.dx.data_ptr() == dy.data_ptr() and lk.dx.shape == dy.shape
    if lk is not None:
        lk.dx = None
    return masked


def _wgrad_stream(device):
    if os.environ.get("RP_WGRAD_OVERLAP", "1") == "0" or torch.cuda.is_current_stream_capturing():
        return None
    return _side2_stream(device)


class _EmbedGatherLinear(torch.autograd.Function):

    @staticmethod
    def forward(ctx, store, idx, dense, ldx: int, weight, bias, out_link, shadow, *tables):
        pre = store._presorted
        store._presorted = None
        need_grad = any(ctx.needs_input_grad[8:])
        need_w = ctx.needs_input_grad[4] or (bias is not None and ctx.needs_input_grad[5])
        B, K, Kg = idx[0].shape[0], weight.shape[1], len(idx) * store.embedding_dim
        wt = None
        if need_grad and weight.is_cuda and weight.dtype is torch.float32 and K % 4 != 0 and K > 64:
            with torch.no_grad():
                wt, w16 = hip.transpose_copy(weight.detach(), rows_out=ldx, ld_copy=(K + 3) // 4 * 4)
        else:
            w16 = _rows16(weight)
        ctx.wt = wt
        if shadow is not None:
            want_keys = pre is None
            seg16 = (need_grad and need_w and K > Kg and len(idx) <= 64 and os.environ.get("RP_GRAD_SEG", "1") != "0"
                     and weight.shape[0] == 64 and store.embedding_dim == 64)
            x, h1, fm, ssum, keys = hip.embed_gather_linear_fwd_bf16(shadow, store.row_base, store.row_count, idx, dense, w16, bias,
                                                                     store.err_flag, train_ldx=ldx, want_keys=want_keys,
                                                                     dense_only=seg16)
            ctx.store, ctx.B, ctx.K, ctx.out_link, ctx.has_bias = store, B, K, out_link, bias is not None
            ctx.ldx, ctx.x_mode, ctx.Kg, ctx.need_tables = ldx, ("seg" if seg16 else "bf16"), Kg, need_grad
            ctx.presorted = pre if need_grad else None
            if pre is not None:
                keys = pre.keys
            ctx.save_for_backward(keys, ssum, x, h1, weight)
            store._fm_link = None
            return h1, fm
        if not need_w:
            x_mode = "none"
        elif (need_grad and K > Kg and len(idx) <= 64 and os.environ.get("RP_GRAD_SEG", "1") != "0"
              and store.embedding_dim == 64 and weight.shape[0] == 64):
            x_mode = "seg"
        else:
            x_mode = "full"
        want_keys = need_grad and pre is None
        x, h1, fm, ssum, keys = hip.embed_gather_linear_fwd(store.arena, store.row_base, store.row_count, idx, dense, ldx, w16,
                                                            bias, True, need_grad, want_keys, store.err_flag,
                                                            x_mode="dense" if x_mode == "seg" else x_mode)
        ctx.store, ctx.B, ctx.K, ctx.out_link, ctx.has_bias = store, B, K, out_link, bias is not None
        ctx.ldx, ctx.x_mode, ctx.Kg, ctx.need_tables = ldx, x_mode, Kg, need_grad
        ctx.presorted = pre if need_grad else None
        if pre is not None:
            keys = pre.keys if need_grad else None
        ctx.save_for_backward(keys, ssum, x, h1, weight)
        store._fm_link = None
        return h1, fm

    @staticmethod
    def backward(ctx, dh1, dfm):
        keys, ssum, x, h1, weight = ctx.saved_tensors
        store = ctx.store
        dh1 = _unit_inner(dh1)
        dpre = dh1 if _masked_by_consumer(ctx.out_link, dh1) else hip.relu_bwd(dh1, h1)
        dw = db = None
        need_w = ctx.needs_input_grad[4] or (ctx.has_bias and ctx.needs_input_grad[5])
        need_t = keys is not None and ctx.need_tables
        if need_w and ctx.x_mode == "none":
            raise RuntimeError("the fused lookup + first layer stored no activation (the forward ran without gradients for the "
                               "layer's weight)")
        seg = need_w and ctx.x_mode == "seg"
        dw_seg = torch.empty((64, ctx.K), dtype=torch.float32, device=dpre.device) if seg else None

        def wgrad():
            if ctx.x_mode == "seg":
                return dw_seg, hip.linear_wgrad(dpre, x, ctx.K - ctx.Kg, dw=dw_seg[:, ctx.Kg:], want_bias=ctx.has_bias)[1]
            if ctx.x_mode == "bf16":
                return hip.linear_wgrad_xbf16(dpre, x, ctx.K, want_bias=ctx.has_bias)
            return hip.linear_wgrad(dpre, x, ctx.K, want_bias=ctx.has_bias)

        wstream = _wgrad_stream(dpre.device) if (need_w and need_t) else None
        plan = hip.LaunchPlan
        in_plan = (wstream is None and need_w and need_t
                   and os.environ.get("RP_WGRAD_OVERLAP", "1") != "0" and plan.is_recording())

        def side_wgrad():
            with plan.side2(in_plan):
                out = wgrad()
                if in_plan:
                    plan.run_deferred()
            return out

        with hip.holding() if in_plan else contextlib.nullcontext():
            if wstream is not None:
                main = torch.cuda.current_stream(dpre.device)
                wstream.wait_stream(main)
                with torch.cuda.stream(wstream):
                    dw, db = wgrad()
            elif need_w and not (in_plan and seg):
                dw, db = side_wgrad()
            if need_t:
                wt = ctx.wt if ctx.wt is not None else hip.transpose(weight, rows_out=ctx.ldx)
                gfm = dfm.contiguous() if dfm is not None else None
                g = store.first_layer_grad(keys, ctx.B, dpre, wt, gfm, ssum if gfm is not None else None, presorted=ctx.presorted,
                                           w=weight if seg else None, dw=dw_seg)
                f = g.forms
                if not seg:
                    if f.tiny:
                        with plan.side2(in_plan):
                            g.tiny()
                    g.gemm()
                elif not in_plan:
                    if f.tiny:
                        g.tiny()
                    ws = g.big(1) if f.big else None
                    if f.rest:
                        g.rest()
                    if f.big:
                        g.big(2, ws)
                else:
                    if f.tiny or not f.big:
                        plan.fork2_mark()
                    if f.big:
                        ws = g.big(1)
                        if f.tiny:
                            with plan.side2():
                                g.tiny()
                            plan.side2_sync()
                        else:
                            plan.fork2_mark()
                    if f.rest:
                        g.rest()
# ... 554 lines not shown
```

### rec_pangu_amd/hip.py

```python
import contextlib
import ctypes as C
import os
import re
from typing import List, Optional, Sequence

import torch

_HERE = os.path.dirname(os.path.abspath(__file__))
HEADER_PATH = os.path.join(_HERE, os.pardir, "include", "rec_pangu_hip.h")
LIB_PATH = os.environ.get("RP_LIB_PATH") or os.path.join(_HERE, "lib", "librecpangu_hip.so")

_lib = None

_i64, _i32, _f32, _vp, _sz = C.c_int64, C.c_int, C.c_float, C.c_void_p, C.c_size_t
_f64 = C.c_double
_C_TYPES = {"int": C.c_int, "int32_t": C.c_int, "int64_t": C.c_int64, "uint32_t": C.c_uint32, "uint64_t": C.c_uint64,
            "size_t": C.c_size_t, "float": C.c_float, "double": C.c_double, "rp_stream_t": C.c_void_p}
_PROTOTYPE = re.compile(r"([A-Za-z_][\w\s]*?[\s*]+)(rp_[a-z0-9_]+)\s*\(([^()]*)\)\s*;")


def parse_header(text: str):
    text = re.sub(r"/\*.*?\*/", " ", text, flags=re.S)
    text = re.sub(r"//[^\n]*", " ", text)
    consts = {m.group(1): int(m.group(2), 0) for m in re.finditer(
# ... 208 lines not shown
    def __init__(self, name, tag=None, nbytes=0, flops=0):
        self.name = name
        self.key = name if tag is None else f"{name}[{tag}]"
        self.meta = (nbytes, flops)

    def __enter__(self):
        self.ev = None
        if _timing is not None and not _timing_paused and (_timing_only is None or self.name in _timing_only):
            self.ev = (torch.cuda.Event(enable_timing=True), torch.cuda.Event(enable_timing=True))
            self.ev[0].record()
        return self

    def __exit__(self, *exc):
        if self.ev is not None:
            self.ev[1].record()
            _timing.setdefault(self.key, []).append(self.ev)
            if self.meta != (0, 0):
                _timing_meta[self.key] = self.meta
        return False


_timing_meta = {}


def timing_summary():
    out = {}
    for name, evs in (_timing or {}).items():
        ms = [a.elapsed_time(b) for a, b in evs]
        out[name] = (len(ms), sum(ms) / max(len(ms), 1))
    return out


def timing_meta():
    return dict(_timing_meta)


_PTR_ARRAYS: dict = {}


def _ptr_array(tensors: Sequence[torch.Tensor]):
    ptrs = tuple([t.data_ptr() for t in tensors])
    arr = _PTR_ARRAYS.get(ptrs)
    if arr is None:
        for i, t in enumerate(tensors):
            if not t.is_cuda:
                raise RuntimeError(f"Expected all tensors to be on the same device: input {i} is on {t.device} but the "
                                   "model is on the HIP device (move the batch with .to(device))")
        arr = (C.c_void_p * max(len(ptrs), 1))(*ptrs)
        if len(_PTR_ARRAYS) >= 512:
            _PTR_ARRAYS.clear()
        _PTR_ARRAYS[ptrs] = arr
    return arr


def embed_gather_fwd(arena, row_base, row_count, idx: List[torch.Tensor], dense: List[torch.Tensor], ldx: int,
                     want_fm: bool, want_sum: bool, want_keys: bool, err_flag: torch.Tensor):
    _req(arena, torch.float32, "arena")
    F, ND = len(idx), len(dense)
    B, D = idx[0].shape[0], arena.shape[1]
    for t in idx:
        _req(t, torch.int64, "index")
        if t.dim() != 1 or t.shape[0] != B or not t.is_contiguous():
            raise RuntimeError("index tensors must be contiguous int64 [B]")
    for t in dense:
        _req(t, torch.float32, "dense")
        if t.dim() != 1 or t.shape[0] != B or not t.is_contiguous():
            raise RuntimeError("dense tensors must be contiguous float32 [B]")
    dev = arena.device
    x = _new((B, ldx), torch.float32, dev)
    fm = _new((B, 1), torch.float32, dev) if want_fm else None
    ssum = _new((B, D), torch.float32, dev) if want_sum else None
    keys = _new((F * B,), torch.int32, dev) if want_keys else None
    with _Timed("embed_gather_fwd", f"D={D}"):
        _check(lib().rp_embed_gather_fwd(arena.data_ptr(), row_base.data_ptr(), row_count.data_ptr(), _ptr_array(idx), F,
                                     _ptr_array(dense), ND, B, D, x.data_ptr(), ldx, _ptr(fm), _ptr(ssum), _ptr(keys),
                                     err_flag.data_ptr(), _stream()), "rp_embed_gather_fwd")
    return x, fm, ssum, keys


def embed_gather_linear_fits(D: int, F: int, ND: int, hidden: int, ldx: int, W) -> bool:
    return F <= 32 and bool(lib().rp_embed_gather_linear_fits(D, ND, hidden, ldx, _rowmajor(W, "W"))) and W.data_ptr() % 16 == 0


def embed_gather_linear_fwd(arena, row_base, row_count, idx: List[torch.Tensor], dense: List[torch.Tensor], ldx: int, W, bias,
                            want_fm: bool, want_sum: bool, want_keys: bool, err_flag: torch.Tensor, x_mode: str = "full"):
    _req(arena, torch.float32, "arena")
    _req(W, torch.float32, "W")
    F, ND = len(idx), len(dense)
    B, D = idx[0].shape[0], arena.shape[1]
    for t in idx:
        _req(t, torch.int64, "index")
        if t.dim() != 1 or t.shape[0] != B or not t.is_contiguous():
            raise RuntimeError("index tensors must be contiguous int64 [B]")
    for t in dense:
        _req(t, torch.float32, "dense")
        if t.dim() != 1 or t.shape[0] != B or not t.is_contiguous():
            raise RuntimeError("dense tensors must be contiguous float32 [B]")
    dev = arena.device
    assert x_mode in ("full", "dense", "none")
    x = _new((B, ldx), torch.float32, dev) if x_mode == "full" else None
    xd = _new((B, 64), torch.float32, dev) if x_mode == "dense" else None
    h1 = _new((B, 64), torch.float32, dev)
    fm = _new((B, 1), torch.float32, dev) if want_fm else None
    ssum = _new((B, D), torch.float32, dev) if want_sum else None
    keys = _new((F * B,), torch.int32, dev) if want_keys else None
    K = F * D + ND
    with _Timed("embed_gather_linear_fwd", f"D={D}", B * (F * (D * 4 + 8) + (F * D + ND) * 4 + 64 * 4), 2 * B * K * 64):
        _check(lib().rp_embed_gather_linear_fwd(arena.data_ptr(), row_base.data_ptr(), row_count.data_ptr(), _ptr_array(idx), F,
                                                _ptr_array(dense), ND, B, D, _ptr(x), ldx, W.data_ptr(), _rowmajor(W, "W"),
                                                _ptr(bias), h1.data_ptr(), _ptr(fm), _ptr(ssum), _ptr(keys),
                                                err_flag.data_ptr(), _ptr(xd), _stream()), "rp_embed_gather_linear_fwd")
    return (x if x_mode == "full" else xd), h1, fm, ssum, keys


def embed_gather_linear_fwd_bf16(arena_bf16, row_base, row_count, idx: List[torch.Tensor], dense: List[torch.Tensor], W, bias,
                                 err_flag: torch.Tensor, train_ldx: int = 0, want_keys: bool = False, dense_only: bool = False):
    _req(arena_bf16, torch.bfloat16, "arena_bf16")
    _req(W, torch.float32, "W")
    F, ND = len(idx), len(dense)
    B, D = idx[0].shape[0], arena_bf16.shape[1]
    dev = arena_bf16.device
    h1 = _new((B, 64), torch.float32, dev)
    fm = _new((B, 1), torch.float32, dev)
    K = F * D + ND
    if train_ldx:
        x16 = None if dense_only else _new((B, train_ldx), torch.bfloat16, dev)
        xd = _new((B, 64), torch.float32, dev) if dense_only else None
        ssum = _new((B, D), torch.float32, dev)
        keys = _new((F * B,), torch.int32, dev) if want_keys else None
        with _Timed("embed_gather_linear_fwd_bf16", f"D={D}", B * (F * (D * 2 + 8) + (F * D + ND) * 2 + 64 * 4 + D * 4), 2 * B * K * 64):
            _check(lib().rp_embed_gather_linear_fwd_bf16(arena_bf16.data_ptr(), row_base.data_ptr(), row_count.data_ptr(),
                                                         _ptr_array(idx), F, _ptr_array(dense), ND, B, D, W.data_ptr(),
                                                         _rowmajor(W, "W"), _ptr(bias), h1.data_ptr(), fm.data_ptr(),
                                                         _ptr(x16), train_ldx, ssum.data_ptr(), _ptr(keys),
                                                         err_flag.data_ptr(), _ptr(xd), _stream()), "rp_embed_gather_linear_fwd_bf16")
        return (xd if dense_only else x16), h1, fm, ssum, keys
    with _Timed("embed_gather_linear_fwd_bf16", f"D={D}", B * (F * (D * 2 + 8) + F * D * 2 + 64 * 4), 2 * B * K * 64):
        _check(lib().rp_embed_gather_linear_fwd_bf16(arena_bf16.data_ptr(), row_base.data_ptr(), row_count.data_ptr(),
                                                     _ptr_array(idx), F, _ptr_array(dense), ND, B, D, W.data_ptr(),
                                                     _rowmajor(W, "W"), _ptr(bias), h1.data_ptr(), fm.data_ptr(),
                                                     None, 0, None, None, err_flag.data_ptr(), None, _stream()),
               "rp_embed_gather_linear_fwd_bf16")
    return h1, fm


def sort_workspace(n: int, device) -> torch.Tensor:
    return _workspace("sort", n, device=device)[0]


def sort_pairs(keys: torch.Tensor, end_bit: int = 32, out=None, workspace=None):
    _req(keys, torch.int32, "keys")
    n = keys.numel()
    ws, nbytes = _workspace("sort", n, device=keys.device, given=workspace)
    assert workspace is None or ws is workspace
    ko, po = (_new_like(keys) if t is None else t for t in (out or (None, None)))
    assert ko.shape == keys.shape and po.shape == keys.shape and ko.dtype == po.dtype == torch.int32
    with _Timed("sort_pairs_i32"):
        _check(lib().rp_sort_pairs_i32(ws.data_ptr(), nbytes, keys.data_ptr(), ko.data_ptr(), po.data_ptr(), n,
                                   end_bit, _stream()), "rp_sort_pairs_i32")
    return ko, po


METRIC_AUC, METRIC_LOGLOSS = _RP["RP_METRIC_AUC"], _RP["RP_METRIC_LOGLOSS"]
METRICS_STAGES = {s: _RP["RP_METRICS_STAGE_" + s.upper()]
                  for s in ("key", "sort", "tile_sums", "tile_scan", "group_neg", "rank", "finish")}


def metrics_workspace(n: int, device) -> torch.Tensor:
    return _workspace("metrics", n, device=device)[0]


def metrics_stage_bytes(n: int, flags: int = METRIC_AUC | METRIC_LOGLOSS) -> dict:
    T = -(-n // 4096)
    auc = bool(flags & METRIC_AUC)
    out = {"key": n * (8 + (4 if auc else 0)) + 20 * T, "finish": (20 + (8 if auc else 0)) * T + 40}
    if auc:
        out.update({"sort": n * 4 * (4 * 2 + 3 + 4 * 2), "tile_sums": n * (4 + 4 + 4 + 1) + 8 * T, "tile_scan": 16 * T,
                    "group_neg": n * (4 + 1 + 4) + 8 * T, "rank": n * (4 + 1 + 4) + 12 * T})
    return out


def binary_metrics(pred: torch.Tensor, label: torch.Tensor, flags: int = METRIC_AUC | METRIC_LOGLOSS, eps: float = 1e-7,
                   workspace=None, result=None, stages=None) -> torch.Tensor:
    _req(pred, torch.float32, "pred")
    _req(label, torch.float32, "label")
    n = pred.numel()
    if label.numel() != n or not pred.is_contiguous() or not label.is_contiguous():
        raise RuntimeError("binary_metrics: pred and label must be contiguous and of one length")
    ws, _ = _workspace("metrics", n, device=pred.device, given=workspace)
    res = _new((5,), torch.int64, pred.device) if result is None else result
    sizes = metrics_stage_bytes(n, flags)
    for tag, bits in ([(None, 0)] if stages is None else [(s, METRICS_STAGES[s]) for s in stages]):
        with _Timed("binary_metrics", tag, sizes.get(tag, 0) if tag else sum(sizes.values())):
            _check(lib().rp_binary_metrics(ws.data_ptr(), ws.numel(), pred.data_ptr(), label.data_ptr(), n, eps, flags | bits,
                                           res.data_ptr(), _stream()), "rp_binary_metrics")
    return res


_SORT_FIELDS: dict = {}


def sort_fields_workspace(B: int, F: int, device) -> torch.Tensor:
    return _workspace("sort_pairs_fields", B, F, device=device)[0]


def sort_pairs_fields(keys: torch.Tensor, B: int, field_rows, out=None, workspace=None):
    _req(keys, torch.int32, "keys")
    F = len(field_rows)
    assert keys.numel() == F * B
    ck = tuple(int(r) for r in field_rows)
    arrs = _SORT_FIELDS.get(ck)
    if arrs is None:
        if len(_SORT_FIELDS) > 64:
            _SORT_FIELDS.clear()
        base, acc = [], 0
        for r in ck:
            base.append(acc)
            acc += r
        arrs = _SORT_FIELDS[ck] = ((C.c_int64 * F)(*base), (C.c_int64 * F)(*ck))
    ws, _ = _workspace("sort_pairs_fields", B, F, device=keys.device, given=workspace)
    ko, po = (_new_like(keys) if t is None else t for t in (out or (None, None)))
    assert ko.shape == keys.shape and po.shape == keys.shape and ko.dtype == po.dtype == torch.int32
    with _Timed("sort_pairs_i32"):
# ... 205 lines not shown
    _req(w, torch.float32, "w")
    lda, ldw = _rowmajor(a, "a"), _rowmajor(w, "w")
    M, N = a.shape[0], w.shape[0]
    K = w.shape[1] if K is None else K
    if a.shape[1] < K:
        raise RuntimeError(f"linear_fwd: a has {a.shape[1]} columns, need {K}")
    if out is None:
        out = _new((M, N), torch.float32, a.device)
    ldo = _rowmajor(out, "out")
    ldaux = _rowmajor(aux, "aux") if aux is not None else 0
    with _Timed("linear_fwd", f"{M}x{N}x{K}", 4 * (M * K + N * K + M * N * (2 if aux is not None else 1)), 2 * M * N * K):
        _check(lib().rp_linear_fwd(a.data_ptr(), lda, w.data_ptr(), ldw, _ptr(bias), out.data_ptr(), ldo, M, N, K, act,
                               _ptr(aux), ldaux, _stream()), "rp_linear_fwd")
    return out


def linear_fwd_rowadd(a, w, row_scale, row_add, add_cols: int, out) -> bool:
    M, K = a.shape
    N = w.shape[0]
    if not (get_matmul_precision() != "fp32" and K <= 64 and K % 4 == 0 and M % 128 == 0 and M >= 128 and N % 64 == 0
            and add_cols % 64 == 0 and 0 < add_cols <= N and row_add.shape[1] == 64 and a.stride(0) % 4 == 0
            and w.stride(0) % 4 == 0 and a.data_ptr() % 16 == 0 and w.data_ptr() % 16 == 0 and out.shape[1] >= N):
        return False
    with _Timed("linear_fwd", f"{M}x{N}x{K}+rowadd", 4 * (M * K + N * K + M * N + M * 65), 2 * M * N * K):
        _check(lib().rp_linear_fwd_rowadd(a.data_ptr(), _rowmajor(a, "a"), w.data_ptr(), _rowmajor(w, "w"), out.data_ptr(),
                                          _rowmajor(out, "out"), M, N, K, row_scale.data_ptr(), row_add.data_ptr(),
                                          _rowmajor(row_add, "row_add"), add_cols, _stream()), "rp_linear_fwd_rowadd")
    return True


def linear_wgrad(dy, x, K: int, dw=None, db=None, accumulate: bool = False, want_bias: bool = True):
    _req(dy, torch.float32, "dy")
    _req(x, torch.float32, "x")
    M, N = dy.shape
    lddy, ldx = _rowmajor(dy, "dy"), _rowmajor(x, "x")
    if dw is None:
        dw = _new((N, K), torch.float32, dy.device)
    if db is None and want_bias:
        db = _new((N,), torch.float32, dy.device)
    ws, nbytes = _workspace("linear_wgrad", M, N, K, device=dy.device)
    with _Timed("linear_wgrad", f"{M}x{N}x{K}", 4 * (M * N + M * K + N * K), 2 * M * N * K):
        _check(lib().rp_linear_wgrad(dy.data_ptr(), lddy, x.data_ptr(), ldx, dw.data_ptr(), _rowmajor(dw, "dw"), _ptr(db),
                                 M, N, K, int(accumulate), ws.data_ptr(), nbytes, _stream()), "rp_linear_wgrad")
    return dw, db


def linear_wgrad_xbf16(dy, x16, K: int, want_bias: bool = True):
    _req(dy, torch.float32, "dy")
    _req(x16, torch.bfloat16, "x16")
    M, N = dy.shape
    dw = _new((N, K), torch.float32, dy.device)
    db = _new((N,), torch.float32, dy.device) if want_bias else None
    ws, nbytes = _workspace("linear_wgrad", M, N, K, device=dy.device)
    with _Timed("linear_wgrad_xbf16", f"{M}x{N}x{K}", 4 * (M * N + N * K) + 2 * M * K, 2 * M * N * K):
        _check(lib().rp_linear_wgrad_xbf16(dy.data_ptr(), _rowmajor(dy, "dy"), x16.data_ptr(), _rowmajor(x16, "x16"),
                                           dw.data_ptr(), K, _ptr(db), M, N, K, 0, ws.data_ptr(), nbytes, _stream()),
               "rp_linear_wgrad_xbf16")
    return dw, db


def transpose(w, rows_out: Optional[int] = None):
    _req(w, torch.float32, "w")
    R, Cc = w.shape
    R4 = (R + 3) // 4 * 4
    rows = max(Cc, rows_out or 0)
    out = _new((rows, R4), torch.float32, w.device)[:, :R]
    with _Timed("transpose", f"{R}x{Cc}", 4 * (R * Cc + rows * R)):
        _check(lib().rp_transpose(w.data_ptr(), _rowmajor(w, "w"), out.data_ptr(), R4, R, Cc, rows, _stream()),
               "rp_transpose")
    return out


def transpose_copy(w, rows_out: int, ld_copy: int):
    _req(w, torch.float32, "w")
    R, Cc = w.shape
    R4 = (R + 3) // 4 * 4
    rows = max(Cc, rows_out or 0)
    out = _new((rows, R4), torch.float32, w.device)[:, :R]
    buf = _new((R, ld_copy), torch.float32, w.device)
    with _Timed("transpose_copy", f"{R}x{Cc}", 4 * (2 * R * Cc + rows * R)):
        _check(lib().rp_transpose_copy(w.data_ptr(), _rowmajor(w, "w"), out.data_ptr(), R4, R, Cc, rows, buf.data_ptr(), ld_copy,
                                       _stream()), "rp_transpose_copy")
    return out, buf[:, :Cc]


def pieces_ld(K: int, np_: int) -> int:
    return int(lib().rp_pieces_ld(int(K), int(np_)))


def pieces_pack(x, np_: int = 2, K: Optional[int] = None, out=None):
    _req(x, torch.float32, "x")
    M = x.shape[0]
    K = x.shape[1] if K is None else K
    ldo = pieces_ld(K, np_)
    if out is None:
        out = _new((M, ldo), torch.bfloat16, x.device)
    with _Timed("pieces_pack", f"{M}x{K}x{np_}", 4 * M * K + 2 * M * ldo):
        _check(lib().rp_pieces_pack(x.data_ptr(), _rowmajor(x, "x"), M, K, np_, out.data_ptr(), _rowmajor(out, "out"), _stream()),
               "rp_pieces_pack")
    return out


def linear_fwd_pieces(a_pc, w_pc, bias, K: int, np_: int = 2, act: int = ACT_NONE, aux=None, out=None):
    _req(a_pc, torch.bfloat16, "a_pc")
    _req(w_pc, torch.bfloat16, "w_pc")
    M, N = a_pc.shape[0], w_pc.shape[0]
    if out is None:
        out = _new((M, N), torch.float32, a_pc.device)
    ldaux = _rowmajor(aux, "aux") if aux is not None else 0
    with _Timed("linear_fwd_pieces", f"{M}x{N}x{K}x{np_}", 2 * (M + N) * pieces_ld(K, np_) + 4 * M * N * (2 if aux is not None else 1),
                2 * M * N * K):
        _check(lib().rp_linear_fwd_pieces(a_pc.data_ptr(), _rowmajor(a_pc, "a_pc"), w_pc.data_ptr(), _rowmajor(w_pc, "w_pc"),
                                          _ptr(bias), out.data_ptr(), _rowmajor(out, "out"), M, N, K, np_, act, _ptr(aux), ldaux,
                                          _stream()), "rp_linear_fwd_pieces")
    return out


def copy_rows(w, ld_out: int):
    _req(w, torch.float32, "w")
    R, Cc = w.shape
    buf = _new((R, ld_out), torch.float32, w.device)
    with _Timed("copy_rows", f"{R}x{Cc}", 8 * R * Cc):
        _check(lib().rp_copy_rows(w.data_ptr(), _rowmajor(w, "w"), buf.data_ptr(), ld_out, R, Cc, _stream()), "rp_copy_rows")
    return buf[:, :Cc]


def copy_rows_to(src, dst):
    _req(src, torch.float32, "src")
    _req(dst, torch.float32, "dst")
    if src.dim() != 2 or src.shape != dst.shape or src.stride(1) != 1 or dst.stride(1) != 1:
        raise RuntimeError("copy_rows_to: two 2-D tensors of one shape with unit inner stride")
    R, Cc = src.shape
    with _Timed("copy_rows", f"{R}x{Cc}", 8 * R * Cc):
        _check(lib().rp_copy_rows(src.data_ptr(), src.stride(0), dst.data_ptr(), dst.stride(0), R, Cc, _stream()), "rp_copy_rows")
    return dst


def add_rows_to(src, dst):
    _req(src, torch.float32, "src")
    _req(dst, torch.float32, "dst")
    if src.dim() != 2 or src.shape != dst.shape or src.stride(1) != 1 or dst.stride(1) != 1:
        raise RuntimeError("add_rows_to: two 2-D tensors of one shape with unit inner stride")
    R, Cc = src.shape
    with _Timed("add_rows", f"{R}x{Cc}", 12 * R * Cc):
        _check(lib().rp_add_rows(src.data_ptr(), src.stride(0), dst.data_ptr(), dst.stride(0), R, Cc, _stream()), "rp_add_rows")
    return dst


class Marker:

    def __init__(self):
        h = _vp()
        _check(lib().rp_marker_create(C.byref(h)), "rp_marker_create")
        self._h = h

    def record(self):
        _check(lib().rp_marker_record(self._h, _stream()), "rp_marker_record")

    def synchronize(self):
        _check(lib().rp_marker_wait(self._h), "rp_marker_wait")

    def __del__(self):
        try:
            if self._h is not None:
                lib().rp_marker_destroy(self._h)
        except Exception:
# ... 2149 lines not shown
```

### rec_pangu_amd/models/layers/embedding.py

```python
import copy
import os
import weakref
from types import SimpleNamespace
from typing import Dict, List, NamedTuple, Optional, Union

import torch
from torch import nn

from ... import functional as Fh
from ...grad_arena import GradArena


class SortedLookup:
    __slots__ = ("keys", "sk", "sp", "src", "versions", "sig", "event", "pinned", "workspace", "want_marks",
                 "smp_sig", "smp", "ss")

    def __init__(self, keys, sk, sp, src=None, sig=None, event=None, pinned=False, workspace=None, want_marks=True):
        self.keys, self.sk, self.sp, self.src, self.sig, self.event = keys, sk, sp, src, sig, event
        self.versions = None if src is None else tuple(t._version for t in src)
        self.pinned, self.workspace, self.want_marks = pinned, workspace, want_marks
        self.smp_sig = self.smp = self.ss = None

    def matches(self, src, sig) -> bool:
        return (self.sig == sig and len(self.src) == len(src) and all(a is b for a, b in zip(self.src, src))
# ... 381 lines not shown
            t = X[c]
            if t.dtype is not torch.int64 or t.dim() != 1 or not t.is_contiguous():
                t = t.long().reshape(-1).contiguous()
            out.append(t)
        return out

    def gather_concat(self, X, dense: List[torch.Tensor], want_fm: bool, pad_to: int = 64):
        self._ensure_packed()
        return self._gather(self._idx_list(X), None, dense, want_fm, pad_to, src=tuple(X[c] for c in self.emb_feature))

    def gather_linear_fits(self, n_dense: int, linear: nn.Linear, pad_to: int = 64) -> bool:
        from ... import hip
        F, D = len(self.emb_feature), self.embedding_dim
        d = F * D + n_dense
        ldx = Fh.padded(d, pad_to)
        w = linear.weight
        key = (id(w), w.data_ptr() % 16, tuple(w.shape), F, D, n_dense, pad_to, self._arena.is_cuda, hip.get_matmul_precision())
        hit = self.__dict__.get("_glf_cache")
        if hit is not None and hit[0] == key:
            return hit[1]
        ok = (self._arena.is_cuda and D == 64 and linear.out_features == 64 and linear.in_features == d
              and hip.get_matmul_precision() != "fp32"
              and hip.embed_gather_linear_fits(D, F, n_dense, 64, ldx, Fh._rows16(w)))
        self.__dict__["_glf_cache"] = (key, ok)
        return ok

    def bf16_lookup(self, enable: bool = True) -> None:
        if not enable:
            self._arena_bf16 = None
            return
        self._ensure_packed()
        self.flush_lazy()
        self._arena_bf16 = self._arena.detach().to(torch.bfloat16)
        self._bf16_stamp = self._bf16_stamp_now()

    def bf16_training(self, enable: bool = True) -> None:
        if not enable:
            self._shadow = None
            return
        self._ensure_packed()
        if not self._arena.is_cuda or self.embedding_dim != 64:
            raise RuntimeError("bf16_training: a HIP-resident layer with embedding_dim 64 (the fused lookup + first layer)")
        self._shadow_rebuild()

    def _shadow_rebuild(self):
        self.flush_lazy()
        self._shadow = self._arena.detach().to(torch.bfloat16)
        self._shadow_stamp = self._shadow_stamp_now()

    def _shadow_stamp_now(self):
        return (self._arena.data_ptr(), self._arena._version, tuple(p._version for p in self._tables()))

    def _shadow_for_training(self):
        sh = self.__dict__.get("_shadow")
        if sh is None:
            return None
        if sh.device != self._arena.device or sh.shape != self._arena.shape or self._shadow_stamp != self._shadow_stamp_now():
            self._shadow_rebuild()
            sh = self._shadow
        return sh

    def _bf16_stamp_now(self):
        from ... import hip
        return (self._arena._version, None if self._lazy is None else self._lazy.t, hip.weight_epoch(),
                tuple(p._version for p in self._tables()))

    def _bf16_arena_for_inference(self):
        a = self.__dict__.get("_arena_bf16")
        if a is None or torch.is_grad_enabled():
            return None
        stamp = self._bf16_stamp_now()
        if stamp != self._bf16_stamp or a.device != self._arena.device:
            raise RuntimeError("the bf16 snapshot of the embedding tables is stale (the model was trained or moved since "
                               "bf16_lookup()): call bf16_lookup() again, or bf16_lookup(False) to read the fp32 tables")
        return a

    def gather_linear(self, X, dense: List[torch.Tensor], linear: nn.Linear, out_link, pad_to: int = 64):
        self._ensure_packed()
        idx = self._idx_list(X)
        a16 = self._bf16_arena_for_inference()
        if a16 is not None:
            from ... import hip
            dense = [t.float().reshape(-1).contiguous() for t in dense]
            out = hip.embed_gather_linear_fwd_bf16(a16, self.row_base, self.row_count, idx, dense, Fh._rows16(linear.weight),
                                                   linear.bias, self.err_flag)
            if self.check_indices == "sync":
                self.raise_if_bad_index()
            return out
        F, D = len(idx), self.embedding_dim
        d = F * D + len(dense)
        ldx = Fh.padded(d, pad_to)
        dense = [t if (t.dtype is torch.float32 and t.dim() == 1 and t.is_contiguous()) else t.float().reshape(-1).contiguous()
                 for t in dense]
        src = tuple(X[c] for c in self.emb_feature)
        self._presorted = None
        shadow = self._shadow_for_training()
        if self._lazy is not None and self._lazy.t > 0:
            self._presorted = self._sorted_keys(idx, self.row_base, self.row_count, src)
            self._lazy.replay(self, self._presorted.sk)
        elif torch.is_grad_enabled():
            self._presorted = self._sorted_keys(idx, self.row_base, self.row_count, src, lookup_only=True)
        out = Fh.embed_gather_linear(self, idx, dense, ldx, linear.weight, linear.bias, out_link, shadow=shadow)
        self._start_sort_ahead()
        if self.check_indices == "sync":
            self.raise_if_bad_index()
        return out

    def _sorted_keys(self, idx, row_base, row_count, src, lookup_only: bool = False):
        from ... import hip
        sig = self._sort_sig()
        look = _find_sort(src, sig) if src is not None else None
        if look is not None:
            if look.event is not None:
                look.wait_on(torch.cuda.current_stream(self._arena.device))
            return look
        if lookup_only:
            return None
        keys = hip.embed_keys(row_base, row_count, idx, self.err_flag)
        sk, sp = self._sort_pairs(keys) if row_base is self.row_base else hip.sort_pairs(keys, end_bit=self._meta()[3])
        look = SortedLookup(keys, sk, sp, src, sig)
        if row_base is self.row_base and torch.is_grad_enabled():
            self._mark_sorted(look)
        if src is not None:
            self._cache_sort(look)
        return look

    def _sort_sig(self):
        return (self._rows_sig(), str(self._arena.device))

    @staticmethod
    def _cache_sort(look: SortedLookup) -> None:
        _SORT_CACHE.append(look)
        del _SORT_CACHE[:-4]

    def prefetch_sort(self, X) -> None:
        if self._arena.is_cuda and all(X[c].device == self._arena.device for c in self.emb_feature):
            self._ahead = X

    def _start_sort_ahead(self) -> None:
        from ... import hip
        X, self._ahead = self.__dict__.get("_ahead"), None
        if X is None:
            return
        src = tuple(X[c] for c in self.emb_feature)
        look = _find_sort(src, self._sort_sig())
        if look is not None:
            if look.pinned:
                self._sort_into(X, look)
            return
        dev = self._arena.device
        side = _side_stream(dev)
        main = torch.cuda.current_stream(dev)
        side.wait_stream(main)
        with torch.cuda.stream(side):
            idx = self._idx_list(X)
            keys = hip.embed_keys(self.row_base, self.row_count, idx, self._ahead_flag())
            look = SortedLookup(keys, *self._sort_pairs(keys), src, self._sort_sig())
            self._mark_sorted(look)
            look.event = torch.cuda.Event()
            look.event.record(side)
        for t in src:
            t.record_stream(side)
        self._cache_sort(look)

    def _ahead_flag(self):
        if self.check_indices != "sync":
            return self.err_flag
        f = self.__dict__.get("_scratch_flag")
# ... 139 lines not shown
```

### rec_pangu_amd/sharded.py

```python
import os
import weakref
from typing import Dict, List, Optional

import torch
import torch.distributed as dist
from torch import nn

from . import functional as Fh
from .grad_arena import GradArena


_STAGED: dict = {}


def _host_staged(t, group) -> bool:
    if not t.is_cuda:
        return False
    k = id(group)
    if k not in _STAGED:
        _STAGED[k] = dist.get_backend(group) == "gloo"
    return _STAGED[k]


def _recorded(fn, t) -> bool:
# ... 186 lines not shown
        self.served = (i32(world * cap), i32(world * cap))
        self.send = self.recv = [cap] * world
        self.n_unique = self.n_recv = cap * world
        self.n_requests, self.capacity, self.b = n, cap, b


class _ShardedRows(torch.autograd.Function):

    @staticmethod
    def forward(ctx, layer, keys, local_arena):
        dev = local_arena.device
        prepared, layer._prepared = layer._prepared, None
        route, recv_rows, served_sorted = prepared if prepared is not None else (None, None, None)
        if route is None:
            route = _Route(keys, layer)
        if recv_rows is None:
            recv_rows = _a2a(route.local_rows, route.recv, route.send, layer.group, layer.world)
        served = layer._local_gather(recv_rows, served_sorted, mark=bool(ctx.needs_input_grad[2]))
        ctx.presorted = getattr(layer, "_served_sorted", None)
        layer._served_sorted = None
        rows = _a2a_rows(served, route.send, route.recv, layer)
        ctx.layer, ctx.route = layer, route
        ctx.scaled, layer._scaled = layer._scaled, None
        ctx.save_for_backward(recv_rows)
        ctx.mark_non_differentiable(route.slot_of_pair, route.slot_sorted, route.pos_sorted)
        ctx.set_materialize_grads(False)
        layer._route_fm = (route.slot_fm, route.pos_fm)
        return rows, route.slot_of_pair, route.slot_sorted, route.pos_sorted

    @staticmethod
    def backward(ctx, g_rows, *_unused):
        (recv_rows,) = ctx.saved_tensors
        layer, route = ctx.layer, ctx.route
        if g_rows is None:
            return None, None, None
        prescaled = layer.world == 1 or (ctx.scaled is not None and ctx.scaled[0]) or _SEED_SCALED[0]
        g_rows = g_rows.contiguous() if prescaled else (g_rows * (1.0 / layer.world)).contiguous()
        recv_g = _a2a_rows(g_rows, route.recv, route.send, layer)
        layer._local_scatter_add(recv_rows, recv_g, presorted=ctx.presorted)
        return None, None, None


class _RowsToX(torch.autograd.Function):

    @staticmethod
    def forward(ctx, rows, slot_of_pair, dense: List[torch.Tensor], slot_sorted, pos_sorted, b: int, F: int, ldx: int,
                want_fm: bool, err_flag):
        from . import hip
        n, D = rows.shape
        dev = rows.device
        zero, cnt = _const_i64(dev, F, 0), _const_i64(dev, F, n)
        idx = [slot_of_pair[f * b:(f + 1) * b] for f in range(F)]
        x, fm, ssum, _ = hip.embed_gather_fwd(rows, zero, cnt, idx, dense, ldx, want_fm, want_fm, False, err_flag)
        ctx.cfg = (b, F, D, want_fm)
        ctx.save_for_backward(rows, slot_sorted, pos_sorted, ssum)
        return (x, fm) if want_fm else x

    @staticmethod
    def backward(ctx, dx, dfm=None):
        from . import hip
        rows, slot_sorted, pos_sorted, ssum = ctx.saved_tensors
        b, F, D, want_fm = ctx.cfg
        g_rows = hip.zeros(rows.shape, rows.dtype, rows.device)
        gfm = dfm.contiguous() if (want_fm and dfm is not None) else None
        dx = None if dx is None else Fh._unit_inner(dx)
        hip.embed_grad_reduce(slot_sorted, pos_sorted, b, D, dx, gfm, ssum if gfm is not None else None,
                              rows if gfm is not None else None, g_rows, accumulate=False)
        return g_rows, None, None, None, None, None, None, None, None, None


class _RowsToLinear(torch.autograd.Function):

    @staticmethod
    def forward(ctx, rows, slot_of_pair, dense: List[torch.Tensor], slot_sorted, pos_sorted, b: int, F: int, ldx: int,
                weight, bias, out_link, err_flag, scale: float, scaled, fm_lists=None):
        from . import hip
        n, D = rows.shape
        dev = rows.device
        zero, cnt = _const_i64(dev, F, 0), _const_i64(dev, F, n)
        idx = [slot_of_pair[f * b:(f + 1) * b] for f in range(F)]
        K = weight.shape[1]
        seg = (fm_lists is not None and fm_lists[0] is not None and K > F * D and F <= 64 and D == 64 and weight.shape[0] == 64
               and (ctx.needs_input_grad[8] or ctx.needs_input_grad[0]) and os.environ.get("RP_GRAD_SEG", "1") != "0")
        x, h1, fm, ssum, _ = hip.embed_gather_linear_fwd(rows, zero, cnt, idx, dense, ldx, Fh._rows16(weight), bias, True,
                                                         True, False, err_flag, x_mode="dense" if seg else "full")
        ctx.cfg = (b, D, K, bias is not None, out_link, scale, scaled, seg, F)
        if seg:
            slot_sorted, pos_sorted = fm_lists
        ctx.save_for_backward(rows, slot_sorted, pos_sorted, ssum, x, h1, weight)
        return h1, fm

    @staticmethod
    def backward(ctx, dh1, dfm):
        from . import hip
        rows, slot_sorted, pos_sorted, ssum, x, h1, weight = ctx.saved_tensors
        b, D, K, has_bias, lk, scale, scaled, seg, F = ctx.cfg
        dh1 = Fh._unit_inner(dh1)
        dpre = dh1 if Fh._masked_by_consumer(lk, dh1) else hip.relu_bwd(dh1, h1)
        dw = db = None
        if seg:
            Kg = F * D
            dw = torch.empty((64, K), dtype=torch.float32, device=dpre.device)
            _, db = hip.linear_wgrad(dpre, x, K - Kg, dw=dw[:, Kg:], want_bias=has_bias)
            gfm = dfm.contiguous() if dfm is not None else None
            fold = scale != 1.0 and not _SEED_SCALED[0]
            dpre_r, gfm_r = dpre, gfm
            if fold:
                dpre_r = dpre * scale
                gfm_r = None if gfm is None else gfm * scale
                scaled[0] = True
            g_rows = hip.zeros(rows.shape, rows.dtype, rows.device)
            hip.embed_grad_seg(slot_sorted, pos_sorted, b, D, dpre_r, weight, gfm_r, ssum if gfm_r is not None else None, rows,
                               g_rows, accumulate=False, dw=dw)
            if fold:
                dw[:, :Kg].mul_(1.0 / scale)
            if not ctx.needs_input_grad[0]:
                g_rows = None
            return g_rows, None, None, None, None, None, None, None, dw, db, None, None, None, None, None
        if ctx.needs_input_grad[8] or (has_bias and ctx.needs_input_grad[9]):
            dw, db = hip.linear_wgrad(dpre, x, K, want_bias=has_bias)
        g_rows = None
        if ctx.needs_input_grad[0]:
            wt = hip.transpose(weight, rows_out=x.shape[1])
            gfm = dfm.contiguous() if dfm is not None else None
            if scale != 1.0 and not _SEED_SCALED[0]:
                dpre = dpre * scale
                gfm = None if gfm is None else gfm * scale
                scaled[0] = True
            g_rows = hip.zeros(rows.shape, rows.dtype, rows.device)
            hip.embed_grad_gemm(slot_sorted, pos_sorted, b, D, dpre, wt, None, gfm, ssum if gfm is not None else None,
                                rows, g_rows, accumulate=False)
        return g_rows, None, None, None, None, None, None, None, dw, db, None, None, None, None, None


class ShardedEmbeddingLayer(nn.Module):

    def __init__(self, full_layer, world: int, rank: int, group=None):
        super().__init__()
        full_layer._ensure_packed()
        rows = [p.shape[0] for p in full_layer.table_parameters()]
        self._setup(full_layer.enc_dict, full_layer.embedding_dim, list(full_layer.emb_feature), rows, world, rank, group,
                    full_layer.arena.device)
        self.check_indices = full_layer.check_indices
        self.local_arena = nn.Parameter(full_layer.arena.detach()[rank::world].clone())
        self._tag()

    @classmethod
    def from_spec(cls, enc_dict, embedding_dim: int, world: int, rank: int, group=None, device=None):
        self = cls.__new__(cls)
        nn.Module.__init__(self)
        cols = [c for c in enc_dict.keys() if "vocab_size" in enc_dict[c].keys()]
        rows = [enc_dict[c]["vocab_size"] + 1 for c in cols]
        dev = torch.empty(0, device=device).device
        self._setup(enc_dict, embedding_dim, cols, rows, world, rank, group, dev)
        n_local = (self.total_rows - rank + world - 1) // world
        self.local_arena = nn.Parameter(torch.empty((n_local, embedding_dim), device=dev))
        self._tag()
        self.init_tables(nn.init.normal_)
        return self

    def _setup(self, enc_dict, embedding_dim, emb_feature, rows, world, rank, group, device):
        self.enc_dict = enc_dict
        self.embedding_dim = embedding_dim
        self.emb_feature = emb_feature
        self.world, self.rank, self.group = world, rank, group
        self.check_indices = "sync"
        self.wire_dtype = torch.float32
# ... 487 lines not shown
```

Before: 87.25 million.

## Prepack bf16 W pieces once and double-buffer them in a 256-row gather-linear tile

The fused embedding gather + first linear layer kernel no longer splits fp32 W into three bf16 pieces inside every block for every field. It reads a pre-split LDS image produced once per step by a new transpose_copy_pieces kernel. The block tile grows from 128 to 256 rows (512 threads), and W slices are double-buffered in LDS so the next field's weights load during the MFMA work. Per-wave fences replace block barriers for the X tile. This adds an extra launch and buffer for the pieces and doubles LDS use, which may lower occupancy.

```diff
diff --git a/include/rec_pangu_hip.h b/include/rec_pangu_hip.h
--- a/include/rec_pangu_hip.h
+++ b/include/rec_pangu_hip.h
@@ -45,11 +45,12 @@
 int rp_embed_gather_linear_fits(int D, int ND, int hidden, int64_t ldx, int64_t ldw);
 int rp_embed_gather_linear_fwd(const float *arena, const int64_t *row_base, const int64_t *row_count,
                                const int64_t *const *idx_ptrs, int F, const float *const *dense_ptrs, int ND, int64_t B,
-                               int D, float *x, int64_t ldx, const float *W, int64_t ldw, const float *bias, float *h1,
+                               int D, float *x, int64_t ldx, const void *w_pieces, const float *bias, float *h1,
                                float *fm_out, float *sum_out, int32_t *keys_out, int32_t *err_flag, float *xd, rp_stream_t stream);
+size_t rp_gather_linear_pieces_bytes(int F);
 int rp_embed_gather_linear_fwd_bf16(const void *arena_bf16, const int64_t *row_base, const int64_t *row_count,
                                     const int64_t *const *idx_ptrs, int F, const float *const *dense_ptrs, int ND, int64_t B,
-                                    int D, const float *W, int64_t ldw, const float *bias, float *h1, float *fm_out,
+                                    int D, const void *w_pieces, const float *bias, float *h1, float *fm_out,
                                     void *x_bf16, int64_t ldx, float *sum_out, int32_t *keys_out, int32_t *err_flag,
                                     float *xd, rp_stream_t stream);
 
@@ -119,6 +120,8 @@
 int rp_transpose(const float *in, int64_t ldin, float *out, int64_t ldout, int R, int C, int C_out, rp_stream_t stream);
 int rp_transpose_copy(const float *in, int64_t ldin, float *out, int64_t ldout, int R, int C, int C_out, float *copy,
                       int64_t ldcopy, rp_stream_t stream);
+int rp_transpose_copy_pieces(const float *in, int64_t ldin, float *out, int64_t ldout, int R, int C, int C_out, float *copy,
+                             int64_t ldcopy, void *pieces, int F, int ND, rp_stream_t stream);
 int rp_copy_rows(const float *in, int64_t ldin, float *out, int64_t ldout, int R, int C, rp_stream_t stream);
 int rp_add_rows(const float *in, int64_t ldin, float *out, int64_t ldout, int R, int C, rp_stream_t stream);
 int64_t rp_pieces_ld(int K, int np);
diff --git a/profiles/microbench/gather_linear_one.py b/profiles/microbench/gather_linear_one.py
--- /dev/null
+++ b/profiles/microbench/gather_linear_one.py
@@ -0,0 +1,39 @@
+import json
+import os
+import sys
+import torch
+sys.path.insert(0, os.path.join(os.path.dirname(os.path.abspath(__file__)), "..", ".."))
+from rec_pangu_amd import hip
+
+CARD = [1460, 583, 10131227, 2202608, 305, 24, 12517, 633, 3, 93145, 5683, 8351593, 3194, 27, 14992, 5461306,
+        10, 5652, 2173, 4, 7046547, 18, 15, 286181, 105, 142572]
+reps = int(sys.argv[1]) if len(sys.argv) > 1 else 10
+B = int(sys.argv[2]) if len(sys.argv) > 2 else 65536
+mode = sys.argv[3] if len(sys.argv) > 3 else "dense"
+hip.lib()
+dev = torch.device("cuda:0")
+F, ND, D = len(CARD), 13, 64
+K = F * D + ND
+cnt = torch.tensor([c + 1 for c in CARD], dtype=torch.int64)
+base = torch.cumsum(cnt, 0) - cnt
+arena = torch.empty((int(cnt.sum()), D), device=dev).uniform_(-0.05, 0.05)
+g = torch.Generator(device=dev).manual_seed(0)
+w = (torch.randn(64, (K + 3) // 4 * 4, device=dev, generator=g) * 0.02)[:, :K]
+bias = torch.zeros(64, device=dev)
+err = torch.zeros(1, dtype=torch.int32, device=dev)
+base_d, cnt_d = base.to(dev), cnt.to(dev)
+batches = []
+for r in range(reps + 2):
+    idx = [torch.randint(0, c + 1, (B,), device=dev, generator=g) for c in CARD]
+    dense = [torch.rand(B, device=dev, generator=g) for _ in range(ND)]
+    batches.append((idx, dense))
+ev = [(torch.cuda.Event(enable_timing=True), torch.cuda.Event(enable_timing=True)) for _ in batches]
+torch.cuda.synchronize()
+for (idx, dense), (e0, e1) in zip(batches, ev):
+    e0.record()
+    hip.embed_gather_linear_fwd(arena, base_d, cnt_d, idx, dense, (K + 3) // 4 * 4, w, bias, True, True, False, err, x_mode=mode)
+    e1.record()
+torch.cuda.synchronize()
+us = [e0.elapsed_time(e1) * 1e3 for e0, e1 in ev][2:]
+print(json.dumps({"probe": "gather_linear_one", "B": B, "mode": mode, "reps": reps, "mean_us": sum(us) / len(us), "min_us": min(us),
+                  "err_flag": int(err.item())}))
diff --git a/rec_pangu_amd/csrc/common.h b/rec_pangu_amd/csrc/common.h
--- a/rec_pangu_amd/csrc/common.h
+++ b/rec_pangu_amd/csrc/common.h
@@ -98,5 +98,9 @@
 
 int rp_matmul_products(double flops, double bytes);
 
+#define RP_GLP_LD 72
+#define RP_GLP_FIELD (3 * 64 * RP_GLP_LD)
+#define RP_GLP_TAIL (3 * 64 * 16)
+
 int rp_int_grad_reduce_finish(int64_t n, int D, int64_t nb0, char *wbase, float *piece0, int32_t *key0, float *grad_arena,
                               int accumulate, hipStream_t s);
diff --git a/rec_pangu_amd/csrc/embed.hip b/rec_pangu_amd/csrc/embed.hip
--- a/rec_pangu_amd/csrc/embed.hip
+++ b/rec_pangu_amd/csrc/embed.hip
@@ -256,25 +256,34 @@
 
 #define EGL_XLD 68
 #define EGL_KLD 33
+#define EGL_TILE 256
+#define EGL_THREADS (2 * EGL_TILE)
+#define EGL_ONE_LAUNCH_BLOCKS 256
+__device__ __forceinline__ void egl_wave_sync() {
+    __builtin_amdgcn_fence(__ATOMIC_RELEASE, "wavefront");
+    __builtin_amdgcn_wave_barrier();
+    __builtin_amdgcn_fence(__ATOMIC_ACQUIRE, "wavefront");
+}
 template <bool FULL, bool STORE_X = true, bool BF16_ROWS = false>
-__global__ __launch_bounds__(256, 2) void embed_gather_linear_kernel(
+__global__ __launch_bounds__(EGL_THREADS, 2) void embed_gather_linear_kernel(
     const float *__restrict__ arena, const int64_t *__restrict__ row_base, const int64_t *__restrict__ row_count,
     IdxPtrs idx, int F, DensePtrs dense, int ND, int64_t B, int64_t blk0, float *__restrict__ x, int64_t ldx,
-    const float *__restrict__ W, int64_t ldw, const float *__restrict__ bias, float *__restrict__ h1,
+    const __bf16 *__restrict__ wp, const float *__restrict__ bias, float *__restrict__ h1,
     float *__restrict__ fm_out, float *__restrict__ sum_out, int32_t *__restrict__ keys_out, int32_t *__restrict__ err_flag,
     float *__restrict__ xd) {
     constexpr int D = 64;
-    __shared__ __attribute__((aligned(16))) __bf16 Wt[3][64][EG_LD];
-    __shared__ __attribute__((aligned(16))) float Xs[128][EGL_XLD];
-    __shared__ int32_t Ks[128][EGL_KLD];
+    static_assert(EG_LD == RP_GLP_LD, "wp holds the LDS image of a field's W slice");
+    __shared__ __attribute__((aligned(16))) __bf16 Wt[2][3][64][EG_LD];
+    __shared__ __attribute__((aligned(16))) float Xs[EGL_TILE][EGL_XLD];
+    __shared__ int32_t Ks[EGL_TILE][EGL_KLD];
     const int t = threadIdx.x;
     const int wv = t >> 6, l = t & 63, i = l & 31, h = l >> 5;
     const int64_t blk = blk0 + blockIdx.x;
-    const int64_t b = blk * 128 + 32 * wv + i;
+    const int64_t b = blk * EGL_TILE + 32 * wv + i;
     const bool bok = FULL || b < B;
     const int64_t bc = bok ? b : B - 1;
-    const int g = t >> 4, sub = t & 15;
-    const int wd = t >> 2, wc = (t & 3) * 16;
+    const int g = l >> 4, sub = l & 15;
+    const int wr = t >> 3, wc = (t & 7) * 8;
 
     for (int f = h; f < F; f += 2) {
         int64_t id = idx.p[f][bc];
@@ -286,16 +295,16 @@
         Ks[32 * wv + i][f] = (int32_t)key;
         if (keys_out != nullptr && bok) keys_out[(int64_t)f * B + b] = (int32_t)key;
     }
-    __syncthreads();
-    const int g8 = t >> 3, s8 = t & 7;
-    auto row_of = [&](int u) { return BF16_ROWS ? g8 + 32 * (u >> 1) : g + 16 * u; };
+    egl_wave_sync();
+    const int g8 = l >> 3, s8 = l & 7;
+    auto row_of = [&](int u) { return 32 * wv + (BF16_ROWS ? g8 + 8 * (u >> 1) : g + 4 * u); };
     auto col_of = [&](int u) { return BF16_ROWS ? 8 * s8 + 4 * (u & 1) : 4 * sub; };
     auto load_rows = [&](int f, f32x4 (&v)[8]) {
         if (BF16_ROWS) {
 #pragma unroll
             for (int u = 0; u < 4; ++u) {
                 const uint4 w4 = *reinterpret_cast<const uint4 *>(reinterpret_cast<const uint16_t *>(arena) +
-                                                                  (int64_t)Ks[g8 + 32 * u][f] * D + 8 * s8);
+                                                                  (int64_t)Ks[row_of(2 * u)][f] * D + 8 * s8);
                 v[2 * u] = f32x4{__uint_as_float(w4.x << 16), __uint_as_float(w4.x & 0xffff0000u),
                                  __uint_as_float(w4.y << 16), __uint_as_float(w4.y & 0xffff0000u)};
                 v[2 * u + 1] = f32x4{__uint_as_float(w4.z << 16), __uint_as_float(w4.z & 0xffff0000u),
@@ -303,13 +312,17 @@
             }
         } else {
 #pragma unroll
-            for (int u = 0; u < 8; ++u) v[u] = *reinterpret_cast<const f32x4 *>(arena + (int64_t)Ks[g + 16 * u][f] * D + 4 * sub);
+            for (int u = 0; u < 8; ++u) v[u] = *reinterpret_cast<const f32x4 *>(arena + (int64_t)Ks[row_of(u)][f] * D + 4 * sub);
         }
     };
-    auto load_w = [&](int col0, f32x4 (&v)[4]) {
-        const float *src = W + (int64_t)wd * ldw + col0 + wc;
-#pragma unroll
-        for (int u = 0; u < 4; ++u) v[u] = *reinterpret_cast<const f32x4 *>(src + 4 * u);
+    auto load_w = [&](int f, u32x4 (&v)[3]) {
+        const __bf16 *src = wp + (int64_t)f * RP_GLP_FIELD + wr * EG_LD + wc;
+#pragma unroll
+        for (int j = 0; j < 3; ++j) v[j] = *reinterpret_cast<const u32x4 *>(src + j * 64 * EG_LD);
+    };
+    auto put_w = [&](int buf, const u32x4 (&v)[3]) {
+#pragma unroll
+        for (int j = 0; j < 3; ++j) *reinterpret_cast<u32x4 *>(&Wt[buf][j][wr][wc]) = v[j];
     };
     f32x16 acc[2];
 #pragma unroll
@@ -323,19 +336,23 @@
         S[u] = f32x4{0.f, 0.f, 0.f, 0.f};
         q[u] = 0.f;
     }
-    f32x4 cur[8], nxt[8], wq[4], wqn[4];
+    f32x4 cur[8], nxt[8];
+    u32x4 wq[3];
     load_rows(0, cur);
     load_w(0, wq);
+    put_w(0, wq);
+    load_w(F > 1 ? 1 : 0, wq);
     for (int f = 0; f < F; ++f) {
         const int fn = f + 1 < F ? f + 1 : f;
         load_rows(fn, nxt);
-        load_w(fn * D, wqn);
         __syncthreads();
+        put_w((f + 1) & 1, wq);
+        load_w(f + 2 < F ? f + 2 : F - 1, wq);
 #pragma unroll
         for (int u = 0; u < 8; ++u) {
             const int r = row_of(u);
             *reinterpret_cast<f32x4 *>(&Xs[r][col_of(u)]) = cur[u];
-            const int64_t br = blk * 128 + r;
+            const int64_t br = blk * EGL_TILE + r;
             if (STORE_X && (FULL || (x != nullptr && br < B))) {
                 if (BF16_ROWS) {
                     uint2 w2;
@@ -350,20 +367,7 @@
 #pragma unroll
             for (int e = 0; e < 4; ++e) q[u] = __builtin_fmaf(cur[u][e], cur[u][e], q[u]);
         }
-#pragma unroll
-        for (int u = 0; u < 2; ++u) {
-            f32x8 v;
-#pragma unroll
-            for (int e = 0; e < 4; ++e) {
-                v[e] = wq[2 * u][e];
-                v[4 + e] = wq[2 * u + 1][e];
-            }
-            bf16x8 pc[3];
-            bf_split8<3>(v, pc);
-#pragma unroll
-            for (int qq = 0; qq < 3; ++qq) *reinterpret_cast<bf16x8 *>(&Wt[qq][wd][wc + 8 * u]) = pc[qq];
-        }
-        __syncthreads();
+        egl_wave_sync();
 #pragma unroll
         for (int ks = 0; ks < 4; ++ks) {
             const f32x4 v0 = *reinterpret_cast<const f32x4 *>(&Xs[32 * wv + i][ks * 16 + 8 * h]);
@@ -380,7 +384,7 @@
             for (int nt = 0; nt < 2; ++nt) {
                 bf16x8 bq[3];
 #pragma unroll
-                for (int qq = 0; qq < 3; ++qq) bq[qq] = *reinterpret_cast<const bf16x8 *>(&Wt[qq][nt * 32 + i][ks * 16 + 8 * h]);
+                for (int qq = 0; qq < 3; ++qq) bq[qq] = *reinterpret_cast<const bf16x8 *>(&Wt[f & 1][qq][nt * 32 + i][ks * 16 + 8 * h]);
 #pragma unroll
                 for (int pr = 0; pr < 6; ++pr) {
                     if (BF16_ROWS && BfProd<6>::pa(pr) != 0) continue;
@@ -388,25 +392,18 @@
                 }
             }
         }
+        egl_wave_sync();
 #pragma unroll
         for (int u = 0; u < 8; ++u) cur[u] = nxt[u];
-#pragma unroll
-        for (int u = 0; u < 4; ++u) wq[u] = wqn[u];
     }
     if (ND > 0) {
         __syncthreads();
-        {
-#pragma unroll
-            for (int u = 0; u < 4; ++u) {
-                const int e = (t & 3) * 4 + u;
-                const float v = e < ND ? W[(int64_t)wd * ldw + (int64_t)F * D + e] : 0.f;
-                const __bf16 hi = (__bf16)v;
-                const float r1 = v - (float)hi;
-                const __bf16 mid = (__bf16)r1;
-                Wt[0][wd][e] = hi;
-                Wt[1][wd][e] = mid;
-                Wt[2][wd][e] = (__bf16)(r1 - (float)mid);
-            }
+#pragma unroll
+        for (int j = 0; j < 2; ++j) {
+            const int c = t + EGL_THREADS * j;
+            if (c < 384)
+                *reinterpret_cast<u32x4 *>(&Wt[0][c >> 7][(c >> 1) & 63][8 * (c & 1)]) =
+                    *reinterpret_cast<const u32x4 *>(wp + (int64_t)F * RP_GLP_FIELD + 8 * c);
         }
         f32x8 dv;
 #pragma unroll
@@ -444,7 +441,7 @@
         for (int nt = 0; nt < 2; ++nt) {
             bf16x8 bq[3];
 #pragma unroll
-            for (int qq = 0; qq < 3; ++qq) bq[qq] = *reinterpret_cast<const bf16x8 *>(&Wt[qq][nt * 32 + i][8 * h]);
+            for (int qq = 0; qq < 3; ++qq) bq[qq] = *reinterpret_cast<const bf16x8 *>(&Wt[0][qq][nt * 32 + i][8 * h]);
 #pragma unroll
             for (int pr = 0; pr < 6; ++pr)
                 acc[nt] = __builtin_amdgcn_mfma_f32_32x32x16_bf16(a[BfProd<6>::pa(pr)], bq[BfProd<6>::pb(pr)], acc[nt], 0, 0, 0);
@@ -463,14 +460,14 @@
         const float bv = bias != nullptr ? bias[n] : 0.f;
 #pragma unroll
         for (int r = 0; r < 16; ++r) {
-            const int64_t m = blk * 128 + 32 * wv + (r & 3) + 8 * (r >> 2) + 4 * h;
+            const int64_t m = blk * EGL_TILE + 32 * wv + (r & 3) + 8 * (r >> 2) + 4 * h;
             if (FULL || m < B) h1[m * 64 + n] = fmaxf(acc[nt][r] + bv, 0.f);
         }
     }
     if (BF16_ROWS) {
 #pragma unroll
         for (int u = 0; u < 4; ++u) {
-            const int64_t br = blk * 128 + g8 + 32 * u;
+            const int64_t br = blk * EGL_TILE + row_of(2 * u);
             float fmv = -(q[2 * u] + q[2 * u + 1]);
 #pragma unroll
             for (int e = 0; e < 4; ++e) {
@@ -490,7 +487,7 @@
     }
 #pragma unroll
     for (int u = 0; u < 8; ++u) {
-        const int64_t br = blk * 128 + g + 16 * u;
+        const int64_t br = blk * EGL_TILE + row_of(u);
         float fmv = -q[u];
 #pragma unroll
         for (int e = 0; e < 4; ++e) fmv = __builtin_fmaf(S[u][e], S[u][e], fmv);
@@ -507,7 +504,7 @@
 
 static int embed_gather_linear_launch(const float *arena, bool bf16_rows, const int64_t *row_base, const int64_t *row_count,
                                       const int64_t *const *idx_ptrs, int F, const float *const *dense_ptrs, int ND,
-                                      int64_t B, int D, float *x, int64_t ldx, const float *W, int64_t ldw,
+                                      int64_t B, int D, float *x, int64_t ldx, const void *w_pieces,
                                       const float *bias, float *h1, float *fm_out, float *sum_out, int32_t *keys_out,
                                       int32_t *err_flag, float *xd, rp_stream_t stream);
 
@@ -515,40 +512,43 @@
     return (D == 64 && hidden == 64 && ND >= 0 && ND <= 16 && ldx % 4 == 0 && ldw % 4 == 0) ? 1 : 0;
 }
 
+extern "C" size_t rp_gather_linear_pieces_bytes(int F) {
+    return F >= 0 ? ((size_t)F * RP_GLP_FIELD + RP_GLP_TAIL) * sizeof(__bf16) : 0;
+}
+
 extern "C" int rp_embed_gather_linear_fwd(const float *arena, const int64_t *row_base, const int64_t *row_count,
                                           const int64_t *const *idx_ptrs, int F, const float *const *dense_ptrs, int ND,
-                                          int64_t B, int D, float *x, int64_t ldx, const float *W, int64_t ldw,
+                                          int64_t B, int D, float *x, int64_t ldx, const void *w_pieces,
                                           const float *bias, float *h1, float *fm_out, float *sum_out, int32_t *keys_out,
                                           int32_t *err_flag, float *xd, rp_stream_t stream) {
-    return embed_gather_linear_launch(arena, false, row_base, row_count, idx_ptrs, F, dense_ptrs, ND, B, D, x, ldx, W, ldw, bias,
+    return embed_gather_linear_launch(arena, false, row_base, row_count, idx_ptrs, F, dense_ptrs, ND, B, D, x, ldx, w_pieces, bias,
                                       h1, fm_out, sum_out, keys_out, err_flag, xd, stream);
 }
 
 extern "C" int rp_embed_gather_linear_fwd_bf16(const void *arena_bf16, const int64_t *row_base, const int64_t *row_count,
                                                const int64_t *const *idx_ptrs, int F, const float *const *dense_ptrs, int ND,
-                                               int64_t B, int D, const float *W, int64_t ldw, const float *bias, float *h1,
+                                               int64_t B, int D, const void *w_pieces, const float *bias, float *h1,
                                                float *fm_out, void *x_bf16, int64_t ldx, float *sum_out, int32_t *keys_out,
                                                int32_t *err_flag, float *xd, rp_stream_t stream) {
     RP_REQUIRE(x_bf16 == nullptr || (ldx % 4 == 0 && (reinterpret_cast<uintptr_t>(x_bf16) & 7u) == 0),
                "embed_gather_linear_fwd_bf16: the bf16 activation needs ldx %% 4 == 0 and 8-byte alignment");
     return embed_gather_linear_launch(reinterpret_cast<const float *>(arena_bf16), true, row_base, row_count, idx_ptrs, F,
-                                      dense_ptrs, ND, B, D, reinterpret_cast<float *>(x_bf16), ldx, W, ldw, bias, h1, fm_out,
+                                      dense_ptrs, ND, B, D, reinterpret_cast<float *>(x_bf16), ldx, w_pieces, bias, h1, fm_out,
                                       sum_out, keys_out, err_flag, xd, stream);
 }
 
 static int embed_gather_linear_launch(const float *arena, bool bf16_rows, const int64_t *row_base, const int64_t *row_count,
                                       const int64_t *const *idx_ptrs, int F, const float *const *dense_ptrs, int ND,
-                                      int64_t B, int D, float *x, int64_t ldx, const float *W, int64_t ldw,
+                                      int64_t B, int D, float *x, int64_t ldx, const void *w_pieces,
                                       const float *bias, float *h1, float *fm_out, float *sum_out, int32_t *keys_out,
                                       int32_t *err_flag, float *xd, rp_stream_t stream) {
-    RP_REQUIRE(arena && row_base && row_count && idx_ptrs && W && h1 && err_flag, "embed_gather_linear_fwd: null pointer");
+    RP_REQUIRE(arena && row_base && row_count && idx_ptrs && w_pieces && h1 && err_flag, "embed_gather_linear_fwd: null pointer");
     RP_REQUIRE(!(x && xd), "embed_gather_linear_fwd: give x (full activation) or xd (dense columns only), not both");
     RP_REQUIRE(F >= 1 && F <= RP_MAX_FIELDS && B >= 0, "embed_gather_linear_fwd: bad F/B");
     RP_REQUIRE(ND == 0 || dense_ptrs, "embed_gather_linear_fwd: dense_ptrs is null with ND=%d", ND);
     RP_REQUIRE((int64_t)F * B < (int64_t)INT32_MAX, "embed_gather_linear_fwd: F*B overflows int32 positions");
-    if (F > EGL_MAXF || !rp_embed_gather_linear_fits(D, ND, 64, x ? ldx : 4, ldw) || !rp_aligned16(arena) || !rp_aligned16(W) ||
-        (x && (!rp_aligned16(x) || ldx < (int64_t)F * D + ND)) || ldw < (int64_t)F * D + ND ||
-        (sum_out && !rp_aligned16(sum_out)))
+    if (F > EGL_MAXF || !rp_embed_gather_linear_fits(D, ND, 64, x ? ldx : 4, 4) || !rp_aligned16(arena) || !rp_aligned16(w_pieces) ||
+        (x && (!rp_aligned16(x) || ldx < (int64_t)F * D + ND)) || (sum_out && !rp_aligned16(sum_out)))
         return rp_fail(RP_ERR_UNSUPPORTED, "embed_gather_linear_fwd: needs D = 64, a 64-wide layer, ND <= 16, aligned operands");
     if (B == 0) return RP_OK;
     IdxPtrs ip;
@@ -561,36 +561,38 @@
         RP_REQUIRE(dense_ptrs[j], "embed_gather_linear_fwd: dense_ptrs[%d] is null", j);
         dp.p[j] = dense_ptrs[j];
     }
-    const int64_t nfull = B / 128;
-    const int64_t nblk = rp_cdiv(B, 128);
+    int64_t nfull = B / EGL_TILE;
+    const int64_t nblk = rp_cdiv(B, EGL_TILE);
+    if (nblk > nfull && nblk <= EGL_ONE_LAUNCH_BLOCKS) nfull = 0;
     hipStream_t s = (hipStream_t)stream;
+    const __bf16 *wp = reinterpret_cast<const __bf16 *>(w_pieces);
     if (bf16_rows) {
         if (nfull > 0 && x != nullptr)
-            hipLaunchKernelGGL((embed_gather_linear_kernel<true, true, true>), dim3((unsigned)nfull), dim3(256), 0, s, arena,
-                               row_base, row_count, ip, F, dp, ND, B, (int64_t)0, x, ldx, W, ldw, bias, h1, fm_out, sum_out,
+            hipLaunchKernelGGL((embed_gather_linear_kernel<true, true, true>), dim3((unsigned)nfull), dim3(EGL_THREADS), 0, s, arena,
+                               row_base, row_count, ip, F, dp, ND, B, (int64_t)0, x, ldx, wp, bias, h1, fm_out, sum_out,
                                keys_out, err_flag, xd);
         else if (nfull > 0)
-            hipLaunchKernelGGL((embed_gather_linear_kernel<true, false, true>), dim3((unsigned)nfull), dim3(256), 0, s, arena,
-                               row_base, row_count, ip, F, dp, ND, B, (int64_t)0, x, ldx, W, ldw, bias, h1, fm_out, sum_out,
+            hipLaunchKernelGGL((embed_gather_linear_kernel<true, false, true>), dim3((unsigned)nfull), dim3(EGL_THREADS), 0, s, arena,
+                               row_base, row_count, ip, F, dp, ND, B, (int64_t)0, x, ldx, wp, bias, h1, fm_out, sum_out,
                                keys_out, err_flag, xd);
         if (nblk > nfull)
-            hipLaunchKernelGGL((embed_gather_linear_kernel<false, true, true>), dim3((unsigned)(nblk - nfull)), dim3(256), 0, s,
-                               arena, row_base, row_count, ip, F, dp, ND, B, nfull, x, ldx, W, ldw, bias, h1, fm_out, sum_out,
+            hipLaunchKernelGGL((embed_gather_linear_kernel<false, true, true>), dim3((unsigned)(nblk - nfull)), dim3(EGL_THREADS), 0, s,
+                               arena, row_base, row_count, ip, F, dp, ND, B, nfull, x, ldx, wp, bias, h1, fm_out, sum_out,
                                keys_out, err_flag, xd);
         RP_LAUNCH_CHECK("embed_gather_linear_fwd (bf16 rows)");
         return RP_OK;
     }
     if (nfull > 0 && x != nullptr)
-        hipLaunchKernelGGL((embed_gather_linear_kernel<true, true>), dim3((unsigned)nfull), dim3(256), 0, s, arena, row_base,
-                           row_count, ip, F, dp, ND, B, (int64_t)0, x, ldx, W, ldw, bias, h1, fm_out, sum_out, keys_out, err_flag,
+        hipLaunchKernelGGL((embed_gather_linear_kernel<true, true>), dim3((unsigned)nfull), dim3(EGL_THREADS), 0, s, arena, row_base,
+                           row_count, ip, F, dp, ND, B, (int64_t)0, x, ldx, wp, bias, h1, fm_out, sum_out, keys_out, err_flag,
                            xd);
     else if (nfull > 0)
-        hipLaunchKernelGGL((embed_gather_linear_kernel<true, false>), dim3((unsigned)nfull), dim3(256), 0, s, arena, row_base,
-                           row_count, ip, F, dp, ND, B, (int64_t)0, x, ldx, W, ldw, bias, h1, fm_out, sum_out, keys_out, err_flag,
+        hipLaunchKernelGGL((embed_gather_linear_kernel<true, false>), dim3((unsigned)nfull), dim3(EGL_THREADS), 0, s, arena, row_base,
+                           row_count, ip, F, dp, ND, B, (int64_t)0, x, ldx, wp, bias, h1, fm_out, sum_out, keys_out, err_flag,
                            xd);
     if (nblk > nfull)
-        hipLaunchKernelGGL((embed_gather_linear_kernel<false, true>), dim3((unsigned)(nblk - nfull)), dim3(256), 0, s, arena,
-                           row_base, row_count, ip, F, dp, ND, B, nfull, x, ldx, W, ldw, bias, h1, fm_out, sum_out, keys_out,
+        hipLaunchKernelGGL((embed_gather_linear_kernel<false, true>), dim3((unsigned)(nblk - nfull)), dim3(EGL_THREADS), 0, s, arena,
+                           row_base, row_count, ip, F, dp, ND, B, nfull, x, ldx, wp, bias, h1, fm_out, sum_out, keys_out,
                            err_flag, xd);
     RP_LAUNCH_CHECK("embed_gather_linear_fwd");
     return RP_OK;
diff --git a/rec_pangu_amd/csrc/gemm.hip b/rec_pangu_amd/csrc/gemm.hip
--- a/rec_pangu_amd/csrc/gemm.hip
+++ b/rec_pangu_amd/csrc/gemm.hip
@@ -932,8 +932,47 @@
 
 __global__ __launch_bounds__(256) void transpose_kernel(const float *__restrict__ in, int64_t ldin,
                                                         float *__restrict__ out, int64_t ldout, int R, int C, int C_out,
-                                                        float *__restrict__ copy = nullptr, int64_t ldcopy = 0) {
+                                                        float *__restrict__ copy = nullptr, int64_t ldcopy = 0,
+                                                        __bf16 *__restrict__ pieces = nullptr, int PF = 0, int PND = 0,
+                                                        int nbx = 0) {
     __shared__ float tile[32][33];
+    if (pieces != nullptr && (int)blockIdx.x >= nbx) {
+        if (blockIdx.y != 0) return;
+        const int items = PF * 64 * (RP_GLP_LD / 8) + 128;
+        for (int it = ((int)blockIdx.x - nbx) * 256 + (int)threadIdx.x; it < items; it += ((int)gridDim.x - nbx) * 256) {
+            const int f = it / (64 * (RP_GLP_LD / 8));
+            if (f < PF) {
+                const int rem = it - f * (64 * (RP_GLP_LD / 8)), n = rem / (RP_GLP_LD / 8), c = rem - n * (RP_GLP_LD / 8);
+                f32x8 v;
+#pragma unroll
+                for (int e = 0; e < 8; ++e) v[e] = c < 8 ? in[(int64_t)n * ldin + f * 64 + 8 * c + e] : 0.f;
+                bf16x8 pc[3];
+                bf_split8<3>(v, pc);
+#pragma unroll
+                for (int q = 0; q < 3; ++q)
+                    *reinterpret_cast<bf16x8 *>(pieces + ((int64_t)(f * 3 + q) * 64 + n) * RP_GLP_LD + 8 * c) = pc[q];
+            } else {
+                const int j = it - PF * 64 * (RP_GLP_LD / 8), n = j >> 1, hh = j & 1;
+                bf16x8 pc[3];
+#pragma unroll
+                for (int e = 0; e < 8; ++e) {
+                    const int k = 8 * hh + e;
+                    const float v = k < PND ? in[(int64_t)n * ldin + PF * 64 + k] : 0.f;
+                    const __bf16 hi = (__bf16)v;
+                    const float r1 = v - (float)hi;
+                    const __bf16 mid = (__bf16)r1;
+                    pc[0][e] = hi;
+                    pc[1][e] = mid;
+                    pc[2][e] = (__bf16)(r1 - (float)mid);
+                }
+                __bf16 *tail = pieces + (int64_t)PF * 3 * 64 * RP_GLP_LD;
+#pragma unroll
+                for (int q = 0; q < 3; ++q) *reinterpret_cast<bf16x8 *>(tail + (q * 64 + n) * 16 + 8 * hh) = pc[q];
+            }
+        }
+        return;
+    }
+    if (out == nullptr) return;
     const int tx = threadIdx.x & 31, ty = threadIdx.x >> 5;
     const int c0 = blockIdx.x * 32, r0 = blockIdx.y * 32;
 #pragma unroll
@@ -1275,6 +1314,22 @@
     return RP_OK;
 }
 
+extern "C" int rp_transpose_copy_pieces(const float *in, int64_t ldin, float *out, int64_t ldout, int R, int C, int C_out,
+                                        float *copy, int64_t ldcopy, void *pieces, int F, int ND, rp_stream_t stream) {
+    RP_REQUIRE(in && pieces && R == 64 && F >= 1 && F <= RP_MAX_FIELDS && ND >= 0 && ND <= 16 && C == 64 * F + ND && ldin >= C,
+               "transpose_copy_pieces: needs a [64, 64 F + ND] matrix, ND <= 16");
+    RP_REQUIRE(rp_aligned16(pieces), "transpose_copy_pieces: the piece buffer must be 16-byte aligned");
+    RP_REQUIRE(copy == nullptr || out != nullptr, "transpose_copy_pieces: a copy goes with the transpose");
+    RP_REQUIRE(out == nullptr || (C_out >= C && ldout >= R && (copy == nullptr || ldcopy >= C)), "transpose_copy_pieces: bad argument");
+    const int nbx = out ? (int)rp_cdiv(C_out, 32) : 0;
+    const int pbx = (int)rp_cdiv((int64_t)F * 64 * (RP_GLP_LD / 8) + 128, 256);
+    const dim3 grid((unsigned)(nbx + pbx), (unsigned)(out ? rp_cdiv(R, 32) : 1));
+    hipLaunchKernelGGL(transpose_kernel, grid, dim3(256), 0, (hipStream_t)stream, in, ldin, out, ldout, R, C, C_out, copy, ldcopy,
+                       reinterpret_cast<__bf16 *>(pieces), F, ND, nbx);
+    RP_LAUNCH_CHECK("transpose_copy_pieces");
+    return RP_OK;
+}
+
 extern "C" int rp_copy_rows(const float *in, int64_t ldin, float *out, int64_t ldout, int R, int C, rp_stream_t stream) {
     RP_REQUIRE(in && out && R >= 1 && C >= 1 && ldin >= C && ldout >= C, "copy_rows: bad argument");
     int64_t blocks = rp_cdiv((int64_t)R * C, 256);
diff --git a/rec_pangu_amd/functional.py b/rec_pangu_amd/functional.py
--- a/rec_pangu_amd/functional.py
+++ b/rec_pangu_amd/functional.py
@@ -55,6 +55,21 @@
     if not key[3]:
         try:
             w._rp_rows16 = (key, out)
+        except AttributeError:
+            pass
+    return out
+
+
+def _gather_linear_pieces(w: torch.Tensor, F: int, ND: int) -> torch.Tensor:
+    key = (w.data_ptr(), w._version, hip.weight_epoch(), torch.cuda.is_current_stream_capturing(), F, ND)
+    hit = getattr(w, "_rp_glp", None)
+    if hit is not None and hit[0] == key:
+        return hit[1]
+    with torch.no_grad():
+        out = hip.gather_linear_pieces(w.detach(), F, ND)
+    if not key[3]:
+        try:
+            w._rp_glp = (key, out)
         except AttributeError:
             pass
     return out
@@ -1466,19 +1481,19 @@
         need_w = ctx.needs_input_grad[4] or (bias is not None and ctx.needs_input_grad[5])
         B, K, Kg = idx[0].shape[0], weight.shape[1], len(idx) * store.embedding_dim
         wt = None
-        if need_grad and weight.is_cuda and weight.dtype is torch.float32 and K % 4 != 0 and K > 64:
-            with torch.no_grad():
-                wt, w16 = hip.transpose_copy(weight.detach(), rows_out=ldx, ld_copy=(K + 3) // 4 * 4)
-        else:
-            w16 = _rows16(weight)
+        with torch.no_grad():
+            if need_grad and K > 64:
+                wt, _, wp = hip.transpose_copy_pieces(weight.detach(), rows_out=ldx, ld_copy=None, F=len(idx), ND=len(dense))
+            else:
+                wp = _gather_linear_pieces(weight, len(idx), len(dense))
         ctx.wt = wt
         if shadow is not None:
             want_keys = pre is None
             seg16 = (need_grad and need_w and K > Kg and len(idx) <= 64 and os.environ.get("RP_GRAD_SEG", "1") != "0"
                      and weight.shape[0] == 64 and store.embedding_dim == 64)
-            x, h1, fm, ssum, keys = hip.embed_gather_linear_fwd_bf16(shadow, store.row_base, store.row_count, idx, dense, w16, bias,
+            x, h1, fm, ssum, keys = hip.embed_gather_linear_fwd_bf16(shadow, store.row_base, store.row_count, idx, dense, None, bias,
                                                                      store.err_flag, train_ldx=ldx, want_keys=want_keys,
-                                                                     dense_only=seg16)
+                                                                     dense_only=seg16, pieces=wp)
             ctx.store, ctx.B, ctx.K, ctx.out_link, ctx.has_bias = store, B, K, out_link, bias is not None
             ctx.ldx, ctx.x_mode, ctx.Kg, ctx.need_tables = ldx, ("seg" if seg16 else "bf16"), Kg, need_grad
             ctx.presorted = pre if need_grad else None
@@ -1495,9 +1510,9 @@
         else:
             x_mode = "full"
         want_keys = need_grad and pre is None
-        x, h1, fm, ssum, keys = hip.embed_gather_linear_fwd(store.arena, store.row_base, store.row_count, idx, dense, ldx, w16,
+        x, h1, fm, ssum, keys = hip.embed_gather_linear_fwd(store.arena, store.row_base, store.row_count, idx, dense, ldx, None,
                                                             bias, True, need_grad, want_keys, store.err_flag,
-                                                            x_mode="dense" if x_mode == "seg" else x_mode)
+                                                            x_mode="dense" if x_mode == "seg" else x_mode, pieces=wp)
         ctx.store, ctx.B, ctx.K, ctx.out_link, ctx.has_bias = store, B, K, out_link, bias is not None
         ctx.ldx, ctx.x_mode, ctx.Kg, ctx.need_tables = ldx, x_mode, Kg, need_grad
         ctx.presorted = pre if need_grad else None
diff --git a/rec_pangu_amd/hip.py b/rec_pangu_amd/hip.py
--- a/rec_pangu_amd/hip.py
+++ b/rec_pangu_amd/hip.py
@@ -314,11 +314,36 @@
     return F <= 32 and bool(lib().rp_embed_gather_linear_fits(D, ND, hidden, ldx, _rowmajor(W, "W"))) and W.data_ptr() % 16 == 0
 
 
+def _glp_bytes(F: int) -> int:
+    return (F * 3 * 64 * 72 + 3 * 64 * 16) * 2
+
+
+def gather_linear_pieces(W, F: int, ND: int):
+    _req(W, torch.float32, "W")
+    if W.dim() != 2 or W.shape[0] != 64 or W.shape[1] != 64 * F + ND:
+        raise RuntimeError(f"W {tuple(W.shape)}: expected [64, {64 * F + ND}]")
+    pieces = _new((_glp_bytes(F),), torch.uint8, W.device)
+    with _Timed("transpose_copy_pieces", f"64x{W.shape[1]}", 4 * 64 * W.shape[1] + pieces.numel()):
+        _check(lib().rp_transpose_copy_pieces(W.data_ptr(), _rowmajor(W, "W"), None, 0, 64, W.shape[1], W.shape[1], None, 0,
+                                              pieces.data_ptr(), F, ND, _stream()), "rp_transpose_copy_pieces")
+    return pieces
+
+
+def _pieces_of(W, pieces, F: int, ND: int):
+    if pieces is None:
+        return gather_linear_pieces(W, F, ND)
+    _req(pieces, torch.uint8, "pieces")
+    if pieces.numel() != _glp_bytes(F) or not pieces.is_contiguous():
+        raise RuntimeError(f"pieces: {pieces.numel()} bytes, not the operand of {F} fields")
+    return pieces
+
+
 def embed_gather_linear_fwd(arena, row_base, row_count, idx: List[torch.Tensor], dense: List[torch.Tensor], ldx: int, W, bias,
-                            want_fm: bool, want_sum: bool, want_keys: bool, err_flag: torch.Tensor, x_mode: str = "full"):
+                            want_fm: bool, want_sum: bool, want_keys: bool, err_flag: torch.Tensor, x_mode: str = "full",
+                            pieces=None):
     _req(arena, torch.float32, "arena")
-    _req(W, torch.float32, "W")
     F, ND = len(idx), len(dense)
+    pieces = _pieces_of(W, pieces, F, ND)
     B, D = idx[0].shape[0], arena.shape[1]
     for t in idx:
         _req(t, torch.int64, "index")
@@ -339,17 +364,18 @@
     K = F * D + ND
     with _Timed("embed_gather_linear_fwd", f"D={D}", B * (F * (D * 4 + 8) + (F * D + ND) * 4 + 64 * 4), 2 * B * K * 64):
         _check(lib().rp_embed_gather_linear_fwd(arena.data_ptr(), row_base.data_ptr(), row_count.data_ptr(), _ptr_array(idx), F,
-                                                _ptr_array(dense), ND, B, D, _ptr(x), ldx, W.data_ptr(), _rowmajor(W, "W"),
+                                                _ptr_array(dense), ND, B, D, _ptr(x), ldx, pieces.data_ptr(),
                                                 _ptr(bias), h1.data_ptr(), _ptr(fm), _ptr(ssum), _ptr(keys),
                                                 err_flag.data_ptr(), _ptr(xd), _stream()), "rp_embed_gather_linear_fwd")
     return (x if x_mode == "full" else xd), h1, fm, ssum, keys
 
 
 def embed_gather_linear_fwd_bf16(arena_bf16, row_base, row_count, idx: List[torch.Tensor], dense: List[torch.Tensor], W, bias,
-                                 err_flag: torch.Tensor, train_ldx: int = 0, want_keys: bool = False, dense_only: bool = False):
+                                 err_flag: torch.Tensor, train_ldx: int = 0, want_keys: bool = False, dense_only: bool = False,
+                                 pieces=None):
     _req(arena_bf16, torch.bfloat16, "arena_bf16")
-    _req(W, torch.float32, "W")
     F, ND = len(idx), len(dense)
+    pieces = _pieces_of(W, pieces, F, ND)
     B, D = idx[0].shape[0], arena_bf16.shape[1]
     dev = arena_bf16.device
     h1 = _new((B, 64), torch.float32, dev)
@@ -362,15 +388,15 @@
         keys = _new((F * B,), torch.int32, dev) if want_keys else None
         with _Timed("embed_gather_linear_fwd_bf16", f"D={D}", B * (F * (D * 2 + 8) + (F * D + ND) * 2 + 64 * 4 + D * 4), 2 * B * K * 64):
             _check(lib().rp_embed_gather_linear_fwd_bf16(arena_bf16.data_ptr(), row_base.data_ptr(), row_count.data_ptr(),
-                                                         _ptr_array(idx), F, _ptr_array(dense), ND, B, D, W.data_ptr(),
-                                                         _rowmajor(W, "W"), _ptr(bias), h1.data_ptr(), fm.data_ptr(),
+                                                         _ptr_array(idx), F, _ptr_array(dense), ND, B, D, pieces.data_ptr(),
+                                                         _ptr(bias), h1.data_ptr(), fm.data_ptr(),
                                                          _ptr(x16), train_ldx, ssum.data_ptr(), _ptr(keys),
                                                          err_flag.data_ptr(), _ptr(xd), _stream()), "rp_embed_gather_linear_fwd_bf16")
         return (xd if dense_only else x16), h1, fm, ssum, keys
     with _Timed("embed_gather_linear_fwd_bf16", f"D={D}", B * (F * (D * 2 + 8) + F * D * 2 + 64 * 4), 2 * B * K * 64):
         _check(lib().rp_embed_gather_linear_fwd_bf16(arena_bf16.data_ptr(), row_base.data_ptr(), row_count.data_ptr(),
-                                                     _ptr_array(idx), F, _ptr_array(dense), ND, B, D, W.data_ptr(),
-                                                     _rowmajor(W, "W"), _ptr(bias), h1.data_ptr(), fm.data_ptr(),
+                                                     _ptr_array(idx), F, _ptr_array(dense), ND, B, D, pieces.data_ptr(),
+                                                     _ptr(bias), h1.data_ptr(), fm.data_ptr(),
                                                      None, 0, None, None, err_flag.data_ptr(), None, _stream()),
                "rp_embed_gather_linear_fwd_bf16")
     return h1, fm
@@ -742,6 +768,21 @@
         _check(lib().rp_transpose_copy(w.data_ptr(), _rowmajor(w, "w"), out.data_ptr(), R4, R, Cc, rows, buf.data_ptr(), ld_copy,
                                        _stream()), "rp_transpose_copy")
     return out, buf[:, :Cc]
+
+
+def transpose_copy_pieces(w, rows_out: int, ld_copy: Optional[int], F: int, ND: int):
+    _req(w, torch.float32, "w")
+    R, Cc = w.shape
+    if R != 64 or Cc != 64 * F + ND:
+        raise RuntimeError(f"w {tuple(w.shape)}: expected [64, {64 * F + ND}]")
+    rows = max(Cc, rows_out or 0)
+    out = _new((rows, R), torch.float32, w.device)
+    buf = _new((R, ld_copy), torch.float32, w.device) if ld_copy else None
+    pieces = _new((_glp_bytes(F),), torch.uint8, w.device)
+    with _Timed("transpose_copy_pieces", f"{R}x{Cc}", 4 * (2 * R * Cc + rows * R) + pieces.numel()):
+        _check(lib().rp_transpose_copy_pieces(w.data_ptr(), _rowmajor(w, "w"), out.data_ptr(), R, R, Cc, rows, _ptr(buf),
+                                              ld_copy or 0, pieces.data_ptr(), F, ND, _stream()), "rp_transpose_copy_pieces")
+    return out, (None if buf is None else buf[:, :Cc]), pieces
 
 
 def pieces_ld(K: int, np_: int) -> int:
diff --git a/rec_pangu_amd/models/layers/embedding.py b/rec_pangu_amd/models/layers/embedding.py
--- a/rec_pangu_amd/models/layers/embedding.py
+++ b/rec_pangu_amd/models/layers/embedding.py
@@ -487,8 +487,8 @@
         if a16 is not None:
             from ... import hip
             dense = [t.float().reshape(-1).contiguous() for t in dense]
-            out = hip.embed_gather_linear_fwd_bf16(a16, self.row_base, self.row_count, idx, dense, Fh._rows16(linear.weight),
-                                                   linear.bias, self.err_flag)
+            out = hip.embed_gather_linear_fwd_bf16(a16, self.row_base, self.row_count, idx, dense, None, linear.bias, self.err_flag,
+                                                   pieces=Fh._gather_linear_pieces(linear.weight, len(idx), len(dense)))
             if self.check_indices == "sync":
                 self.raise_if_bad_index()
             return out
diff --git a/rec_pangu_amd/sharded.py b/rec_pangu_amd/sharded.py
--- a/rec_pangu_amd/sharded.py
+++ b/rec_pangu_amd/sharded.py
@@ -292,7 +292,7 @@
         K = weight.shape[1]
         seg = (fm_lists is not None and fm_lists[0] is not None and K > F * D and F <= 64 and D == 64 and weight.shape[0] == 64
                and (ctx.needs_input_grad[8] or ctx.needs_input_grad[0]) and os.environ.get("RP_GRAD_SEG", "1") != "0")
-        x, h1, fm, ssum, _ = hip.embed_gather_linear_fwd(rows, zero, cnt, idx, dense, ldx, Fh._rows16(weight), bias, True,
+        x, h1, fm, ssum, _ = hip.embed_gather_linear_fwd(rows, zero, cnt, idx, dense, ldx, weight.detach(), bias, True,
                                                          True, False, err_flag, x_mode="dense" if seg else "full")
         ctx.cfg = (b, D, K, bias is not None, out_link, scale, scaled, seg, F)
         if seg:
```

Result: no change. 87.91 million (median of 6 runs) (+0.8%).
